# unixpickle/vq-voice-swap

Hardware: AMD Instinct MI355X
Metric: audio clips/sec (whole node), unet64 50-step DDPM on 4s@16kHz waveforms (higher is better)
Workload: dtype fp16; 1 GPU; unet64 50-step DDPM (constrain, schedule t**2), 64 clips/GPU x 1 GPU of T=64000; global_batch=64, parallelism=clips sharded over 1 GPU(s), gather to rank 0

## Files before the change

include/vqvs.h:

```cpp
#ifndef VQVS_H
#define VQVS_H

#include <stdint.h>

#ifdef __cplusplus
extern "C" {
#endif

#define VQVS_OK 0
#define VQVS_ERR_ARG (-1)
#define VQVS_ERR_HIP (-2)
#define VQVS_ERR_STATE (-3)

#define VQVS_KIND_PREDICTOR 0
#define VQVS_KIND_ENCODER 1
#define VQVS_KIND_RESBLOCK 2
#define VQVS_KIND_CLASSIFIER 3
#define VQVS_KIND_ENCPRED 4

#define VQVS_KIND_MFCC_ENCODER 5

#define VQVS_KIND_PREDICTOR_GRAD 6

#define VQVS_PREC_F32 0
#define VQVS_PREC_BF16 1
#define VQVS_PREC_F16 2

typedef struct vqvs_model vqvs_model;

typedef struct vqvs_cfg {
  int32_t kind;
  int32_t base_channels;
  int32_t in_channels;
  int32_t out_channels;
  int32_t cond_channels;
  int32_t num_labels;
  int32_t precision;
  int32_t max_batch;
  int32_t max_T;
  int32_t debug_taps;
  int32_t rb_cin, rb_cout, rb_resize , rb_dilation, rb_emb_channels ;
  int32_t reserved[5];
  int32_t topology_set;
  int32_t n_levels;
  int32_t channel_mult[12];
  int32_t depth_mult;
  int32_t n_dilations;
  int32_t dilations[12];
} vqvs_cfg;
#define VQVS_MAX_LEVELS 12

int vqvs_param_count(const vqvs_cfg* cfg);
int vqvs_param_info(const vqvs_cfg* cfg, int index, char* name_out, int name_cap, int64_t shape_out[4], int* ndim_out);

int vqvs_model_create(const vqvs_cfg* cfg, const float* const* h_params, int n_params, int device, vqvs_model** out);
void vqvs_model_destroy(vqvs_model* m);
int64_t vqvs_model_device_bytes(const vqvs_model* m);

int vqvs_unet_forward(vqvs_model* m, const float* d_x, const float* d_ts, const float* d_cond,
                      const int64_t* d_labels, float* d_out, int B, int T, void* stream);

int vqvs_encoder_forward(vqvs_model* m, const float* d_x, float* d_z, int B, int T, void* stream);

int vqvs_mfcc_encoder_forward(vqvs_model* m, const float* d_x, float* d_z, int B, int T, void* stream);

int vqvs_mfcc_encoder_forward_logmel(vqvs_model* m, const float* d_logmel, float* d_z, int B, int T, void* stream);

int vqvs_resblock_forward(vqvs_model* m, const float* d_x, const float* d_emb, float* d_y, int B, int L, void* stream);

int vqvs_model_status(vqvs_model* m, unsigned* h_status);

int vqvs_classifier_forward(vqvs_model* m, const float* d_x, const float* d_ts, float* d_logits, int B, int T, void* stream);
int vqvs_classifier_guidance(vqvs_model* m, const float* d_x, const float* d_ts, const int64_t* d_labels, float scale,
                             float* d_grad, float* d_logits, int B, int T, void* stream);
int vqvs_classifier_features(vqvs_model* m, const float* d_x, const float* d_ts, float* d_feat,
                             float* d_logits, float* d_probs, int B, int T, void* stream);

int vqvs_feature_moments(const float* d_feat, int B, int F, const float* d_shift, double* d_s1, double* d_s2, void* stream);

int vqvs_encpred_forward(vqvs_model* m, const float* d_x, const float* d_ts, float* d_logits, int B, int T, void* stream);
int vqvs_encpred_guidance(vqvs_model* m, const float* d_x, const float* d_ts, const int64_t* d_targets, float scale,
                          float* d_grad, float* d_logits, int B, int T, void* stream);

int vqvs_unet_embed_grad(vqvs_model* m, const float* d_x_t, const float* d_ts, const float* d_cond, const float* d_vec,
                         const float* d_eps, float* d_mse, float* d_grad, float* d_pred, int B, int T, void* stream);
int vqvs_embed_adamw(float* d_rows, float* d_m, float* d_v, const float* d_grad, const int64_t* d_row_of_clip, int n, int B, int E,
                     int step, float lr, float beta1, float beta2, float eps, float weight_decay, void* stream);

int vqvs_head_xent_grad(const float* d_feat, const float* d_w_old, const float* d_b_old, const float* d_new, const int64_t* d_targets,
                        float* d_act, float* d_logits, double* d_nll, int64_t* d_top1, double* d_new_mass, double* d_coef, int B, int F,
                        int K, int n, void* stream);
int vqvs_head_adamw(float* d_new, float* d_m, float* d_v, const float* d_act, const double* d_coef, int n, int B, int F, int step,
                    float lr, float beta1, float beta2, float eps, float weight_decay, void* stream);

#define VQVS_DDPM_SIGMA_LARGE 1u
#define VQVS_DDPM_CONSTRAIN 2u
int vqvs_ddpm_step(const float* d_x_t, const float* d_eps, const float* d_noise, const float* d_alpha_t,
                   const float* d_alpha_prev, float* d_x_prev, int B, int T, uint32_t flags, float noise_scale,
                   uint64_t seed, uint64_t clip_offset, uint32_t step_index, void* stream);
int vqvs_ddpm_step_windows(const float* d_x, const float* d_eps, const float* d_noise, const float* d_alpha_t,
                           const float* d_alpha_prev, float* d_x_prev, float* d_windows, int n, int W, int H, uint32_t flags,
                           float noise_scale, uint64_t seed, uint64_t clip, uint32_t step_index, void* stream);
int vqvs_ddpm_mean(const float* d_x_t, const float* d_eps, const float* d_alpha_t, const float* d_alpha_prev,
                   float* d_mean, int B, int T, void* stream);
int vqvs_ddpm_guided_eps(const float* d_x_t, const float* d_mean, const float* d_grad, const float* d_alpha_t,
                         const float* d_alpha_prev, float* d_eps_out, int B, int T, uint32_t flags, void* stream);
#define VQVS_DDIM_CONSTRAIN 2u
#define VQVS_DDIM_INVERT 4u
int vqvs_ddim_step(const float* d_x_t, const float* d_eps, const float* d_grad, const float* d_noise, const float* d_alpha_t,
                   const float* d_alpha_to, float* d_x_to, int B, int T, uint32_t flags, float eta, float noise_scale,
                   uint64_t seed, uint64_t clip_offset, uint32_t step_index, void* stream);
int vqvs_ddim_step_windows(const float* d_x, const float* d_eps, const float* d_grad, const float* d_noise, const float* d_alpha_t,
                           const float* d_alpha_to, float* d_x_to, float* d_windows, int n, int W, int H, uint32_t flags, float eta,
                           float noise_scale, uint64_t seed, uint64_t clip, uint32_t step_index, void* stream);
int vqvs_dpmpp_step(const float* d_x_t, const float* d_eps, const float* d_grad, const float* d_x0_prev, const float* d_alpha_from,
                    const float* d_alpha_t, const float* d_alpha_to, float* d_x_to, float* d_x0_out, int B, int T, uint32_t flags,
                    void* stream);
int vqvs_dpmpp_step_windows(const float* d_x, const float* d_eps, const float* d_grad, const float* d_x0_prev, const float* d_alpha_from,
                            const float* d_alpha_t, const float* d_alpha_to, float* d_x_to, float* d_x0_out, float* d_windows, int n, int W,
                            int H, uint32_t flags, void* stream);
int vqvs_keep_region(float* d_x, const float* d_x0, const uint8_t* d_keep, const float* d_noise, const float* d_alpha, int B, int T,
                     float noise_scale, uint64_t seed, uint64_t clip_offset, uint32_t index, void* stream);
int vqvs_keep_region_windows(float* d_x, float* d_windows, const float* d_x0, const uint8_t* d_keep, const float* d_noise,
                             const float* d_alpha, int n, int W, int H, float noise_scale, uint64_t seed, uint64_t clip, uint32_t index,
                             void* stream);
int vqvs_randn(float* d_out, int B, int T, uint64_t seed, uint64_t clip_offset, uint32_t stream_id, void* stream);

int vqvs_ddpm_noise(const float* d_x0, int x0_rows, const float* d_alpha, const float* d_eps, int eps_rows,
                    const int64_t* d_noise_index, float* d_x_t, int B, int T, uint64_t seed, uint64_t clip_offset, void* stream);
int vqvs_ddpm_sqerr(const float* d_pred, const float* d_eps, int eps_rows, const int64_t* d_noise_index, float* d_loss,
                    int B, int T, uint64_t seed, uint64_t clip_offset, void* stream);

int vqvs_vq_argmin(const float* d_z, const float* d_dict, int64_t* d_idx, int B, int Cd, int T1, int K, void* stream);
int vqvs_vq_quantize(const float* d_z, const float* d_dict, int64_t* d_idx, float* d_embedded, double* d_sqerr, int64_t* d_hist,
                     int B, int Cd, int T1, int K, void* stream);
int vqvs_vq_embed(const int64_t* d_idx, const float* d_dict, float* d_out, int B, int Cd, int T1, int K, void* stream);

int vqvs_xent_score(const float* d_logits, const int64_t* d_targets, double* d_nll, int64_t* d_top1, int64_t* d_topk, int k,
                    int64_t* d_confusion, int B, int K, int L, void* stream);

int vqvs_spectral_distance(const float* d_a, const float* d_b, const float* d_window, const double* d_twiddle,
                           const float* d_fb, const float* d_dct, double* d_mcd, double* d_lsd,
                           int B, int T, int n_fft, int hop, int n_mels, int n_ceps, float eps, void* stream);
// ... 27 lines not shown
```

vq_voice_swap_amd/_native.py:

```python

from __future__ import annotations

import ctypes as C
import os
import subprocess
from typing import Dict, List, Optional, Sequence, Tuple

_HERE = os.path.dirname(os.path.abspath(__file__))
LIB_PATH = os.environ.get("VQVS_LIB_PATH") or os.path.join(_HERE, "libvqvs_hip.so")
CSRC = os.path.join(_HERE, "csrc")

KIND_PREDICTOR, KIND_ENCODER, KIND_RESBLOCK, KIND_CLASSIFIER, KIND_ENCPRED, KIND_MFCC_ENCODER, KIND_PREDICTOR_GRAD = 0, 1, 2, 3, 4, 5, 6
PREC_F32, PREC_BF16, PREC_F16 = 0, 1, 2
DDPM_SIGMA_LARGE, DDPM_CONSTRAIN = 1, 2
DDIM_CONSTRAIN, DDIM_INVERT = 2, 4
STREAM_STEP, STREAM_XT, STREAM_LOSS, STREAM_KEEP = 0, 1, 2, 3
PRECISIONS = {"fp32": PREC_F32, "f32": PREC_F32, "float32": PREC_F32, "bf16": PREC_BF16, "bfloat16": PREC_BF16,
              "fp16": PREC_F16, "f16": PREC_F16, "float16": PREC_F16, "half": PREC_F16}


class Cfg(C.Structure):
    _fields_ = [
        ("kind", C.c_int32),
        ("base_channels", C.c_int32),
        ("in_channels", C.c_int32),
        ("out_channels", C.c_int32),
        ("cond_channels", C.c_int32),
        ("num_labels", C.c_int32),
        ("precision", C.c_int32),
        ("max_batch", C.c_int32),
        ("max_T", C.c_int32),
        ("debug_taps", C.c_int32),
        ("rb_cin", C.c_int32),
        ("rb_cout", C.c_int32),
        ("rb_resize", C.c_int32),
        ("rb_dilation", C.c_int32),
        ("rb_emb_channels", C.c_int32),
        ("reserved", C.c_int32 * 5),
        ("topology_set", C.c_int32),
        ("n_levels", C.c_int32),
        ("channel_mult", C.c_int32 * 12),
        ("depth_mult", C.c_int32),
        ("n_dilations", C.c_int32),
        ("dilations", C.c_int32 * 12),
    ]

    def set_topology(self, channel_mult, depth_mult, dilations):
        if len(channel_mult) > 12 or len(dilations) > 12:
            raise ValueError("the gfx950 library builds at most 12 levels and 12 middle / output dilations")
        self.topology_set = 1
        self.n_levels = len(channel_mult)
        for i, m in enumerate(channel_mult):
            self.channel_mult[i] = int(m)
        self.depth_mult = int(depth_mult)
        self.n_dilations = len(dilations)
        for i, d in enumerate(dilations):
            self.dilations[i] = int(d)


EXPORTS = [
    "vqvs_param_count", "vqvs_param_info", "vqvs_model_create", "vqvs_model_destroy", "vqvs_model_device_bytes",
    "vqvs_unet_forward", "vqvs_encoder_forward", "vqvs_mfcc_encoder_forward", "vqvs_mfcc_encoder_forward_logmel", "vqvs_model_status", "vqvs_resblock_forward", "vqvs_classifier_forward",
    "vqvs_classifier_guidance", "vqvs_classifier_features", "vqvs_feature_moments", "vqvs_encpred_forward", "vqvs_encpred_guidance", "vqvs_ddpm_step", "vqvs_ddpm_step_windows", "vqvs_ddim_step", "vqvs_ddim_step_windows", "vqvs_dpmpp_step", "vqvs_dpmpp_step_windows", "vqvs_keep_region", "vqvs_keep_region_windows", "vqvs_ddpm_mean",
    "vqvs_ddpm_guided_eps", "vqvs_randn", "vqvs_ddpm_noise", "vqvs_ddpm_sqerr", "vqvs_vq_argmin", "vqvs_vq_quantize", "vqvs_vq_embed", "vqvs_xent_score", "vqvs_spectral_distance", "vqvs_pitch_distance", "vqvs_debug_tap_count",
    "vqvs_debug_tap_info", "vqvs_debug_tap_rows", "vqvs_debug_read_tap", "vqvs_debug_read_embedding", "vqvs_forward_kernel_count", "vqvs_forward_model_bytes",
    "vqvs_forward_flops", "vqvs_set_profiling", "vqvs_op_info", "vqvs_op_desc", "vqvs_profile_read", "vqvs_last_error", "vqvs_version",
    "vqvs_unet_embed_grad", "vqvs_embed_adamw", "vqvs_debug_read_dfilm", "vqvs_head_xent_grad", "vqvs_head_adamw",
]

_lib = None


class NativeError(RuntimeError):
    pass


class NativeArgumentError(NativeError, ValueError):
    """VQVS_ERR_ARG: the library refused the arguments on the host, before it touched the device.  A ValueError, as the
    reference raises for shape problems, and a NativeError like every other error the library reports."""


def build(force: bool = False, verbose: bool = False) -> str:
    cmd = ["make", "-C", CSRC, "-j", str(min(8, os.cpu_count() or 1))]
    if force:
        subprocess.run(["make", "-C", CSRC, "clean"], check=True, capture_output=not verbose)
    r = subprocess.run(cmd, capture_output=True, text=True)
    if r.returncode != 0:
        raise NativeError("building libvqvs_hip.so failed:\n" + r.stdout[-4000:] + r.stderr[-4000:])
    if verbose:
        print(r.stdout)
    return LIB_PATH


def lib():
    global _lib
    if _lib is not None:
        return _lib
    if not os.path.exists(LIB_PATH):
        raise NativeError(
            f"{LIB_PATH} is missing. Build it with `python -c 'import __graft_entry__ as g; g.build()'` "
            "(or `make -C vq_voice_swap_amd/csrc`). There is no CPU fallback for the sampling hot path."
        )
    if os.environ.get("HIP_FORCE_DEV_KERNARG") is None:
        import warnings

        warnings.warn("HIP_FORCE_DEV_KERNARG is not set: the HIP runtime keeps kernel arguments in host memory and every launch of the "
                      "sampler starts with loads across PCIe (~2 % slower, DESIGN.md section 7).  Set HIP_FORCE_DEV_KERNARG=1 in the "
                      "process environment before the first HIP call (bench.py and the sample_*.py scripts do).", RuntimeWarning, stacklevel=2)
    L = C.CDLL(LIB_PATH)
    vp, i32, i64, u32, u64, f32 = C.c_void_p, C.c_int, C.c_int64, C.c_uint32, C.c_uint64, C.c_float
    L.vqvs_last_error.restype = C.c_char_p
    L.vqvs_version.restype = C.c_char_p
    L.vqvs_param_count.argtypes = [C.POINTER(Cfg)]
    L.vqvs_param_info.argtypes = [C.POINTER(Cfg), i32, C.c_char_p, i32, C.POINTER(i64), C.POINTER(i32)]
    L.vqvs_model_create.argtypes = [C.POINTER(Cfg), C.POINTER(vp), i32, i32, C.POINTER(vp)]
    L.vqvs_model_destroy.argtypes = [vp]
    L.vqvs_model_destroy.restype = None
    L.vqvs_model_device_bytes.argtypes = [vp]
    L.vqvs_model_device_bytes.restype = i64
    L.vqvs_unet_forward.argtypes = [vp, vp, vp, vp, vp, vp, i32, i32, vp]
    L.vqvs_unet_embed_grad.argtypes = [vp, vp, vp, vp, vp, vp, vp, vp, vp, i32, i32, vp]
    L.vqvs_embed_adamw.argtypes = [vp, vp, vp, vp, vp, i32, i32, i32, i32, f32, f32, f32, f32, f32, vp]
    L.vqvs_debug_read_dfilm.argtypes = [vp, i32, vp]
    L.vqvs_head_xent_grad.argtypes = [vp, vp, vp, vp, vp, vp, vp, vp, vp, vp, vp, i32, i32, i32, i32, vp]
    L.vqvs_head_adamw.argtypes = [vp, vp, vp, vp, vp, i32, i32, i32, i32, f32, f32, f32, f32, f32, vp]
    L.vqvs_encoder_forward.argtypes = [vp, vp, vp, i32, i32, vp]
    L.vqvs_mfcc_encoder_forward.argtypes = [vp, vp, vp, i32, i32, vp]
    L.vqvs_mfcc_encoder_forward_logmel.argtypes = [vp, vp, vp, i32, i32, vp]
    L.vqvs_model_status.argtypes = [vp, vp]
    L.vqvs_resblock_forward.argtypes = [vp, vp, vp, vp, i32, i32, vp]
    L.vqvs_classifier_forward.argtypes = [vp, vp, vp, vp, i32, i32, vp]
    L.vqvs_classifier_guidance.argtypes = [vp, vp, vp, vp, f32, vp, vp, i32, i32, vp]
    L.vqvs_classifier_features.argtypes = [vp, vp, vp, vp, vp, vp, i32, i32, vp]
    L.vqvs_feature_moments.argtypes = [vp, i32, i32, vp, vp, vp, vp]
    L.vqvs_encpred_forward.argtypes = [vp, vp, vp, vp, i32, i32, vp]
    L.vqvs_encpred_guidance.argtypes = [vp, vp, vp, vp, f32, vp, vp, i32, i32, vp]
    L.vqvs_ddpm_step.argtypes = [vp, vp, vp, vp, vp, vp, i32, i32, u32, f32, u64, u64, u32, vp]
    L.vqvs_ddpm_step_windows.argtypes = [vp, vp, vp, vp, vp, vp, vp, i32, i32, i32, u32, f32, u64, u64, u32, vp]
    L.vqvs_ddim_step.argtypes = [vp, vp, vp, vp, vp, vp, vp, i32, i32, u32, f32, f32, u64, u64, u32, vp]
    L.vqvs_ddim_step_windows.argtypes = [vp, vp, vp, vp, vp, vp, vp, vp, i32, i32, i32, u32, f32, f32, u64, u64, u32, vp]
    L.vqvs_dpmpp_step.argtypes = [vp, vp, vp, vp, vp, vp, vp, vp, vp, i32, i32, u32, vp]
    L.vqvs_dpmpp_step_windows.argtypes = [vp, vp, vp, vp, vp, vp, vp, vp, vp, vp, i32, i32, i32, u32, vp]
    L.vqvs_keep_region.argtypes = [vp, vp, vp, vp, vp, i32, i32, f32, u64, u64, u32, vp]
    L.vqvs_keep_region_windows.argtypes = [vp, vp, vp, vp, vp, vp, i32, i32, i32, f32, u64, u64, u32, vp]
    L.vqvs_ddpm_mean.argtypes = [vp, vp, vp, vp, vp, i32, i32, vp]
    L.vqvs_ddpm_guided_eps.argtypes = [vp, vp, vp, vp, vp, vp, i32, i32, u32, vp]
    L.vqvs_randn.argtypes = [vp, i32, i32, u64, u64, u32, vp]
    L.vqvs_ddpm_noise.argtypes = [vp, i32, vp, vp, i32, vp, vp, i32, i32, u64, u64, vp]
    L.vqvs_ddpm_sqerr.argtypes = [vp, vp, i32, vp, vp, i32, i32, u64, u64, vp]
    L.vqvs_vq_argmin.argtypes = [vp, vp, vp, i32, i32, i32, i32, vp]
    L.vqvs_vq_quantize.argtypes = [vp, vp, vp, vp, vp, vp, i32, i32, i32, i32, vp]
    L.vqvs_vq_embed.argtypes = [vp, vp, vp, i32, i32, i32, i32, vp]
    L.vqvs_xent_score.argtypes = [vp, vp, vp, vp, vp, i32, vp, i32, i32, i32, vp]
    L.vqvs_spectral_distance.argtypes = [vp, vp, vp, vp, vp, vp, vp, vp, i32, i32, i32, i32, i32, i32, f32, vp]
    L.vqvs_pitch_distance.argtypes = [vp, vp, vp, vp, vp, vp, i32, i32, i32, i32, i32, i32, C.c_double, vp]
    L.vqvs_debug_tap_count.argtypes = [vp]
    L.vqvs_debug_tap_info.argtypes = [vp, i32, C.c_char_p, i32, C.POINTER(i32), C.POINTER(i32)]
    L.vqvs_debug_tap_rows.argtypes = [vp, i32, i32]
    L.vqvs_debug_read_tap.argtypes = [vp, i32, i32, i32, vp]
    L.vqvs_debug_read_embedding.argtypes = [vp, i32, vp]
    L.vqvs_forward_kernel_count.argtypes = [vp]
    L.vqvs_forward_model_bytes.argtypes = [vp, i32, i32]
    L.vqvs_forward_model_bytes.restype = i64
    L.vqvs_forward_flops.argtypes = [vp, i32, i32]
    L.vqvs_forward_flops.restype = i64
    L.vqvs_set_profiling.argtypes = [vp, i32]
    L.vqvs_op_info.argtypes = [vp, i32, C.c_char_p, i32, C.POINTER(i64), C.POINTER(i64), i32, i32]
    L.vqvs_profile_read.argtypes = [vp, vp, i32]
    L.vqvs_op_desc.argtypes = [vp, i32, C.c_char_p, i32]
    _lib = L
    return L


def last_error() -> str:
    return (lib().vqvs_last_error() or b"").decode("utf-8", "replace")


def check(rc: int) -> None:
    if rc == 0:
        return
    msg = last_error()
    if rc == -1:
        if msg.startswith("must provide"):
            raise AssertionError(msg)
        raise NativeArgumentError(msg)
    raise NativeError(f"libvqvs_hip error {rc}: {msg}")


def param_table(cfg: Cfg) -> List[Tuple[str, Tuple[int, ...]]]:
    L = lib()
    n = L.vqvs_param_count(C.byref(cfg))
    if n < 0:
        check(n)
    out = []
    name = C.create_string_buffer(256)
    shape = (C.c_int64 * 4)()
    nd = C.c_int()
    for i in range(n):
        check(L.vqvs_param_info(C.byref(cfg), i, name, 256, shape, C.byref(nd)))
        out.append((name.value.decode(), tuple(int(shape[k]) for k in range(nd.value))))
    return out


# ... 162 lines not shown
```

vq_voice_swap_amd/csrc/api.cpp:

```cpp
#include <cmath>
#include <cstring>
#include <initializer_list>
#include <map>
#include <mutex>
#include <string>
#include <utility>
#include <vector>

#include "net.hpp"
#include "sampler_kernels.hpp"

namespace vqvs {
static thread_local std::string g_err;
void set_error(const std::string& msg) { g_err = msg; }

struct DeviceScratch {
  void* p = nullptr;
  size_t bytes = 0;
  unsigned long long used = 0;
  int leases = 0;
  std::vector<void*> retired;
};
static std::map<std::pair<int, void*>, DeviceScratch> g_scratch;
static std::mutex g_scratch_mu;
// ... 41 lines not shown
      VQVS_HIP(hipFree(sc.p));
      sc.p = nullptr;
      sc.bytes = 0;
    }
  } else if (sc.p && sc.bytes < bytes) {
    sc.retired.push_back(sc.p);
    sc.p = nullptr;
    sc.bytes = 0;
  }
  if (!sc.p) {
    size_t n = bytes < MIN_BYTES ? MIN_BYTES : bytes;
    VQVS_HIP(hipMalloc(&sc.p, n));
    sc.bytes = n;
  }
  sc.used = ++g_scratch_tick;
  ++sc.leases;
  lease.sc = &sc;
  lease.p = sc.p;
  return 0;
}
}

using namespace vqvs;

extern "C" {

const char* vqvs_last_error(void) { return g_err.c_str(); }
#ifndef VQVS_BUILD_ID
#define VQVS_BUILD_ID "unstamped"
#endif
const char* vqvs_version(void) { return "vqvs-hip 0.1 (gfx950) build " VQVS_BUILD_ID; }

int vqvs_param_count(const vqvs_cfg* cfg) {
  if (!cfg) VQVS_FAIL(VQVS_ERR_ARG, "cfg is NULL");
  std::vector<ParamDef> p;
  if (int e = enumerate_params(*cfg, p)) return e;
  return (int)p.size();
}

int vqvs_param_info(const vqvs_cfg* cfg, int index, char* name_out, int name_cap, int64_t shape_out[4], int* ndim_out) {
  if (!cfg) VQVS_FAIL(VQVS_ERR_ARG, "cfg is NULL");
  std::vector<ParamDef> p;
  if (int e = enumerate_params(*cfg, p)) return e;
  if (index < 0 || index >= (int)p.size()) VQVS_FAIL(VQVS_ERR_ARG, "param index %d out of range", index);
  const ParamDef& d = p[index];
  if (name_out && name_cap > 0) {
    strncpy(name_out, d.name.c_str(), name_cap - 1);
    name_out[name_cap - 1] = 0;
  }
  if (shape_out)
    for (int i = 0; i < 4; ++i) shape_out[i] = i < (int)d.shape.size() ? d.shape[i] : 1;
  if (ndim_out) *ndim_out = (int)d.shape.size();
  return 0;
}

int vqvs_model_create(const vqvs_cfg* cfg, const float* const* h_params, int n_params, int device, vqvs_model** out) {
  if (!cfg || !h_params || !out) VQVS_FAIL(VQVS_ERR_ARG, "NULL argument");
  *out = nullptr;
  std::vector<ParamDef> p;
  if (int e = enumerate_params(*cfg, p)) return e;
  if (n_params != (int)p.size()) VQVS_FAIL(VQVS_ERR_ARG, "expected %d parameters, got %d", (int)p.size(), n_params);
  for (int i = 0; i < n_params; ++i)
    if (!h_params[i]) VQVS_FAIL(VQVS_ERR_ARG, "parameter %d (%s) is NULL", i, p[i].name.c_str());
  int ndev = 0;
  VQVS_HIP(hipGetDeviceCount(&ndev));
  if (device < 0 || device >= ndev) VQVS_FAIL(VQVS_ERR_ARG, "device %d not present (%d visible)", device, ndev);
  VQVS_HIP(hipSetDevice(device));
  vqvs_model* m = new vqvs_model();
  m->cfg = *cfg;
  m->device = device;
  if (int e = build_model(m, h_params)) {
    vqvs_model_destroy(m);
    return e;
  }
  *out = m;
  return 0;
}

void vqvs_model_destroy(vqvs_model* m) {
  if (!m) return;
  for (auto e : m->events) (void)hipEventDestroy(e);
  if (m->d_weights) (void)hipFree(m->d_weights);
  if (m->d_arena) (void)hipFree(m->d_arena);
  delete m;
}

int64_t vqvs_model_device_bytes(const vqvs_model* m) { return m ? (int64_t)(m->weights_bytes + m->arena_bytes) : 0; }

static int check_run(vqvs_model* m, int kind, int B, int L) {
  if (!m) VQVS_FAIL(VQVS_ERR_ARG, "model is NULL");
  if (m->cfg.kind != kind) VQVS_FAIL(VQVS_ERR_STATE, "handle kind %d used as kind %d", m->cfg.kind, kind);
  if (B < 1 || B > m->cfg.max_batch) VQVS_FAIL(VQVS_ERR_ARG, "batch %d outside 1..%d", B, m->cfg.max_batch);
  if (L < 1 || L > m->cfg.max_T) VQVS_FAIL(VQVS_ERR_ARG, "length %d outside 1..%d", L, m->cfg.max_T);
  if (kind == VQVS_KIND_CLASSIFIER && (L % (2 * unet_rate(m->cfg))))
    VQVS_FAIL(VQVS_ERR_ARG, "T=%d is not a multiple of the classifier downsample rate %d", L, 2 * unet_rate(m->cfg));
  if (kind != VQVS_KIND_RESBLOCK && kind != VQVS_KIND_MFCC_ENCODER && (L % unet_rate(m->cfg)))
    VQVS_FAIL(VQVS_ERR_ARG, "T=%d is not a multiple of the UNet downsample rate %d", L, unet_rate(m->cfg));
  if (kind == VQVS_KIND_RESBLOCK && m->cfg.rb_resize == RESIZE_AVG2 && (L % 2)) VQVS_FAIL(VQVS_ERR_ARG, "avg-pool resblock needs even L");
  return 0;
}

int vqvs_unet_forward(vqvs_model* m, const float* d_x, const float* d_ts, const float* d_cond, const int64_t* d_labels, float* d_out,
                      int B, int T, void* stream) {
  if (int e = check_run(m, VQVS_KIND_PREDICTOR, B, T)) return e;
  if (!d_x || !d_ts || !d_out) VQVS_FAIL(VQVS_ERR_ARG, "x, ts and out must be non-NULL");
  if ((d_labels == nullptr) != (m->cfg.num_labels == 0)) VQVS_FAIL(VQVS_ERR_ARG, "must provide labels if and only if model is class conditional");
  if ((d_cond == nullptr) != (m->cfg.cond_channels == 0)) VQVS_FAIL(VQVS_ERR_ARG, "must provide cond sequence if and only if model is conditional");
  RunCtx c;
  c.B = B;
  c.Lbase = T;
  c.x = d_x;
  c.ts = d_ts;
  c.cond = d_cond;
  c.labels = d_labels;
  c.out = d_out;
  c.st = reinterpret_cast<hipStream_t>(stream);
  return run_model(m, c);
}

int vqvs_unet_embed_grad(vqvs_model* m, const float* d_x_t, const float* d_ts, const float* d_cond, const float* d_vec, const float* d_eps,
                         float* d_mse, float* d_grad, float* d_pred, int B, int T, void* stream) {
  if (int e = check_run(m, VQVS_KIND_PREDICTOR_GRAD, B, T)) return e;
  if (!d_x_t || !d_ts || !d_vec) VQVS_FAIL(VQVS_ERR_ARG, "x_t, ts and vec must be non-NULL");
  if ((d_cond == nullptr) != (m->cfg.cond_channels == 0)) VQVS_FAIL(VQVS_ERR_ARG, "must provide cond sequence if and only if model is conditional");
  if ((d_mse == nullptr) != (d_grad == nullptr)) VQVS_FAIL(VQVS_ERR_ARG, "mse and grad must be given together (both NULL: the forward alone)");
  const bool backward = d_grad != nullptr;
  if (backward && !d_eps) VQVS_FAIL(VQVS_ERR_ARG, "eps must be non-NULL when mse and grad are asked for");
  if (!backward && !d_pred) VQVS_FAIL(VQVS_ERR_ARG, "nothing to compute: mse, grad and pred are all NULL");
  RunCtx c;
  c.B = B;
  c.Lbase = T;
  c.x = d_x_t;
  c.ts = d_ts;
  c.cond = d_cond;
  c.class_vec = d_vec;
  c.eps = d_eps;
  c.mse = d_mse;
  c.egrad = d_grad;
  c.out = d_pred;
  c.backward = backward;
  c.st = reinterpret_cast<hipStream_t>(stream);
  return run_model(m, c);
}

int vqvs_embed_adamw(float* d_rows, float* d_m, float* d_v, const float* d_grad, const int64_t* d_row_of_clip, int n, int B, int E,
                     int step, float lr, float beta1, float beta2, float eps, float weight_decay, void* stream) {
  if (!d_rows || !d_m || !d_v || !d_grad || !d_row_of_clip) VQVS_FAIL(VQVS_ERR_ARG, "rows, m, v, grad and row_of_clip must be non-NULL");
  if (n < 1 || B < 1 || E < 1) VQVS_FAIL(VQVS_ERR_ARG, "bad shape n=%d B=%d E=%d", n, B, E);
  if (step < 1) VQVS_FAIL(VQVS_ERR_ARG, "step=%d: the count of this step starts at 1", step);
  if (!std::isfinite(lr) || lr < 0.f) VQVS_FAIL(VQVS_ERR_ARG, "lr=%g must be finite and not negative", (double)lr);
  if (!std::isfinite(eps) || eps < 0.f) VQVS_FAIL(VQVS_ERR_ARG, "eps=%g must be finite and not negative", (double)eps);
  if (!std::isfinite(weight_decay) || weight_decay < 0.f) VQVS_FAIL(VQVS_ERR_ARG, "weight_decay=%g must be finite and not negative", (double)weight_decay);
  if (!(beta1 >= 0.f && beta1 < 1.f) || !(beta2 >= 0.f && beta2 < 1.f)) VQVS_FAIL(VQVS_ERR_ARG, "betas (%g, %g) must lie in [0, 1)", (double)beta1, (double)beta2);
  return run_embed_adamw(d_rows, d_m, d_v, d_grad, d_row_of_clip, n, B, E, step, lr, beta1, beta2, eps, weight_decay,
                         reinterpret_cast<hipStream_t>(stream));
}

int vqvs_head_xent_grad(const float* d_feat, const float* d_w_old, const float* d_b_old, const float* d_new, const int64_t* d_targets,
                        float* d_act, float* d_logits, double* d_nll, int64_t* d_top1, double* d_new_mass, double* d_coef, int B, int F,
                        int K, int n, void* stream) {
  if (!d_feat || !d_w_old || !d_b_old || !d_new || !d_targets || !d_nll || !d_coef)
    VQVS_FAIL(VQVS_ERR_ARG, "feat, w_old, b_old, new, targets, nll and coef must be non-NULL");
  if (B < 1 || B > 65535) VQVS_FAIL(VQVS_ERR_ARG, "batch %d outside 1..65535", B);
  if (F < 1 || F > 4096) VQVS_FAIL(VQVS_ERR_ARG, "feature width %d outside 1..4096", F);
  if (K < 1 || n < 1 || K > 8192 || n > 8192 || K + n > 8192) VQVS_FAIL(VQVS_ERR_ARG, "K=%d old and n=%d new labels: each at least 1, together at most 8192", K, n);
  return run_head_xent_grad(d_feat, d_w_old, d_b_old, d_new, d_targets, d_act, d_logits, d_nll, d_top1, d_new_mass, d_coef, B, F, K, n,
                            reinterpret_cast<hipStream_t>(stream));
}

int vqvs_head_adamw(float* d_new, float* d_m, float* d_v, const float* d_act, const double* d_coef, int n, int B, int F, int step,
                    float lr, float beta1, float beta2, float eps, float weight_decay, void* stream) {
  if (!d_new || !d_m || !d_v || !d_act || !d_coef) VQVS_FAIL(VQVS_ERR_ARG, "new, m, v, act and coef must be non-NULL");
  if (n < 1 || B < 1 || F < 1) VQVS_FAIL(VQVS_ERR_ARG, "bad shape n=%d B=%d F=%d", n, B, F);
  if (n > 8192 || B > 65535 || F > 4096) VQVS_FAIL(VQVS_ERR_ARG, "n=%d B=%d F=%d outside 1..8192, 1..65535, 1..4096", n, B, F);
  if (step < 1) VQVS_FAIL(VQVS_ERR_ARG, "step=%d: the count of this step starts at 1", step);
  if (!std::isfinite(lr) || lr < 0.f) VQVS_FAIL(VQVS_ERR_ARG, "lr=%g must be finite and not negative", (double)lr);
  if (!std::isfinite(eps) || eps < 0.f) VQVS_FAIL(VQVS_ERR_ARG, "eps=%g must be finite and not negative", (double)eps);
  if (!std::isfinite(weight_decay) || weight_decay < 0.f) VQVS_FAIL(VQVS_ERR_ARG, "weight_decay=%g must be finite and not negative", (double)weight_decay);
  if (!(beta1 >= 0.f && beta1 < 1.f) || !(beta2 >= 0.f && beta2 < 1.f)) VQVS_FAIL(VQVS_ERR_ARG, "betas (%g, %g) must lie in [0, 1)", (double)beta1, (double)beta2);
  return run_head_adamw(d_new, d_m, d_v, d_act, d_coef, n, B, F, step, lr, beta1, beta2, eps, weight_decay,
                        reinterpret_cast<hipStream_t>(stream));
}

int vqvs_encoder_forward(vqvs_model* m, const float* d_x, float* d_z, int B, int T, void* stream) {
  if (int e = check_run(m, VQVS_KIND_ENCODER, B, T)) return e;
  if (!d_x || !d_z) VQVS_FAIL(VQVS_ERR_ARG, "x and z must be non-NULL");
  RunCtx c;
  c.B = B;
  c.Lbase = T;
  c.x = d_x;
  c.out = d_z;
  c.st = reinterpret_cast<hipStream_t>(stream);
  return run_model(m, c);
}

int vqvs_mfcc_encoder_forward(vqvs_model* m, const float* d_x, float* d_z, int B, int T, void* stream) {
  if (int e = check_run(m, VQVS_KIND_MFCC_ENCODER, B, T)) return e;
  if (!d_x || !d_z) VQVS_FAIL(VQVS_ERR_ARG, "x and z must be non-NULL");
  if (T < 800) VQVS_FAIL(VQVS_ERR_ARG, "T=%d is too short for the MFCC front end (needs at least 800 samples)", T);
// ... 415 lines not shown
  if (!a) VQVS_FAIL(VQVS_ERR_ARG, "a must be non-NULL");
  if (!b && (period_b || counts || sums)) VQVS_FAIL(VQVS_ERR_ARG, "b is NULL: period_b, counts and sums must be NULL too");
  if (!b && !period_a) VQVS_FAIL(VQVS_ERR_ARG, "b is NULL: period_a must be given");
  if (!period_a && !period_b && !counts && !sums) VQVS_FAIL(VQVS_ERR_ARG, "every output is NULL: nothing to compute");
  if (B < 1 || B > 65535) VQVS_FAIL(VQVS_ERR_ARG, "batch %d outside 1..65535", B);
  if (T < 1 || T > (1 << 30)) VQVS_FAIL(VQVS_ERR_ARG, "clip of %d samples outside 1..2^30", T);
  if (window < 16 || window > 2048) VQVS_FAIL(VQVS_ERR_ARG, "window=%d outside 16..2048", window);
  if (hop < 1 || hop > window) VQVS_FAIL(VQVS_ERR_ARG, "hop=%d outside 1..window=%d", hop, window);
  if (T / hop + 1 > (1 << 25)) VQVS_FAIL(VQVS_ERR_ARG, "T=%d at hop=%d is more than 2^25 frames per clip", T, hop);
  if (tau_max < 3 || tau_max > 1023) VQVS_FAIL(VQVS_ERR_ARG, "tau_max=%d outside 3..1023", tau_max);
  if (tau_min < 2 || tau_min >= tau_max) VQVS_FAIL(VQVS_ERR_ARG, "tau_min=%d outside 2..tau_max-1=%d", tau_min, tau_max - 1);
  if ((int64_t)window * tau_max > (1 << 20))
    VQVS_FAIL(VQVS_ERR_ARG, "window=%d times tau_max=%d is more than 2^20: the sums would not stay below 2^53", window, tau_max);
  if (!std::isfinite(threshold) || !(threshold > 0.0) || threshold > 1.0) VQVS_FAIL(VQVS_ERR_ARG, "threshold=%g must lie in (0, 1]", threshold);
  const int64_t N = (int64_t)B * T, NF = (int64_t)B * (T / hop + 1);
  const struct { const void* p; int64_t bytes; const char* name; } outs[] = {
      {period_a, NF * 8, "period_a"}, {period_b, NF * 8, "period_b"}, {counts, (int64_t)B * 32, "counts"}, {sums, (int64_t)B * 16, "sums"}};
  for (const auto& out : outs) {
    if (bytes_overlap(out.p, out.bytes, a, N * 4) || bytes_overlap(out.p, out.bytes, b, N * 4))
      VQVS_FAIL(VQVS_ERR_ARG, "%s must not overlap a or b", out.name);
    for (const auto& other : outs)
      if (&other != &out && bytes_overlap(out.p, out.bytes, other.p, other.bytes))
        VQVS_FAIL(VQVS_ERR_ARG, "%s must not overlap %s", out.name, other.name);
  }
  ScratchLease lease;
  if (counts || sums)
    if (int e = scratch_get(pitch_distance_scratch_bytes(B, T, hop), stream, lease)) return e;
  return run_pitch_distance(a, b, period_a, period_b, counts, sums, lease.p, B, T, window, hop, tau_min, tau_max, threshold,
                            reinterpret_cast<hipStream_t>(stream));
}

int vqvs_vq_embed(const int64_t* d_idx, const float* d_dict, float* d_out, int B, int Cd, int T1, int K, void* stream) {
  if (!d_idx || !d_dict || !d_out) VQVS_FAIL(VQVS_ERR_ARG, "idx, dict and out must be non-NULL");
  if (B < 1 || Cd < 1 || T1 < 1 || K < 1) VQVS_FAIL(VQVS_ERR_ARG, "bad shape B=%d Cd=%d T1=%d K=%d", B, Cd, T1, K);
  if (B > 65535) VQVS_FAIL(VQVS_ERR_ARG, "batch %d outside 1..65535", B);
  if (Cd > 65535) VQVS_FAIL(VQVS_ERR_ARG, "channels %d outside 1..65535", Cd);
  return run_vq_embed(d_idx, d_dict, d_out, B, Cd, T1, K, reinterpret_cast<hipStream_t>(stream));
}

int vqvs_debug_tap_count(const vqvs_model* m) { return m ? (int)m->taps.size() : 0; }

int vqvs_debug_tap_info(const vqvs_model* m, int i, char* name_out, int name_cap, int* channels, int* length_shift) {
  if (!m || i < 0 || i >= (int)m->taps.size()) VQVS_FAIL(VQVS_ERR_ARG, "bad tap index");
  if (name_out && name_cap > 0) {
    strncpy(name_out, m->taps[i].name.c_str(), name_cap - 1);
    name_out[name_cap - 1] = 0;
  }
  if (channels) *channels = m->taps[i].t.C;
  if (length_shift) *length_shift = m->taps[i].t.lshift;
  return 0;
}

int vqvs_debug_tap_rows(const vqvs_model* m, int i, int T) {
  if (!m || i < 0 || i >= (int)m->taps.size()) VQVS_FAIL(VQVS_ERR_ARG, "bad tap index");
  return tensor_rows(T, m->taps[i].t.lshift);
}

int vqvs_debug_read_tap(vqvs_model* m, int i, int B, int T, float* h_out) {
  if (!m || i < 0 || i >= (int)m->taps.size() || !h_out) VQVS_FAIL(VQVS_ERR_ARG, "bad argument");
  if (!m->cfg.debug_taps) VQVS_FAIL(VQVS_ERR_STATE, "model was not created with debug_taps=1");
  const TensorH& t = m->taps[i].t;
  const int L = tensor_rows(T, t.lshift);
  const size_t n = (size_t)B * t.C * L;
  float* d_tmp = nullptr;
  VQVS_HIP(hipSetDevice(m->device));
  VQVS_HIP(hipMalloc(reinterpret_cast<void**>(&d_tmp), n * 4));
  int e = launch_ntc_to_nct(m->d_arena + t.off, d_tmp, B, t.C, L, t.f32 ? 0 : m->cfg.precision, nullptr);
  if (!e) {
    hipError_t he = hipMemcpy(h_out, d_tmp, n * 4, hipMemcpyDeviceToHost);
    if (he != hipSuccess) {
      set_error(std::string("hipMemcpy failed: ") + hipGetErrorString(he));
      e = VQVS_ERR_HIP;
    }
  }
  (void)hipFree(d_tmp);
  return e;
}

int vqvs_debug_read_embedding(vqvs_model* m, int B, float* h_out) {
  if (!m || !h_out || B < 1 || B > m->cfg.max_batch) VQVS_FAIL(VQVS_ERR_ARG, "bad argument");
  if (!m->emb_E) VQVS_FAIL(VQVS_ERR_STATE, "this model kind has no timestep embedding");
  VQVS_HIP(hipSetDevice(m->device));
  VQVS_HIP(hipDeviceSynchronize());
  const float* src = reinterpret_cast<const float*>(m->d_arena + m->misc_off) + m->emb_misc_off;
  VQVS_HIP(hipMemcpy(h_out, src, (size_t)B * m->emb_E * sizeof(float), hipMemcpyDeviceToHost));
  return m->emb_E;
}

int vqvs_debug_read_dfilm(vqvs_model* m, int B, float* h_out) {
  if (!m || !h_out || B < 1 || B > m->cfg.max_batch) VQVS_FAIL(VQVS_ERR_ARG, "bad argument");
  if (!m->dfilm_R) VQVS_FAIL(VQVS_ERR_STATE, "this model kind has no FiLM-gradient buffer");
  VQVS_HIP(hipSetDevice(m->device));
  VQVS_HIP(hipDeviceSynchronize());
  const float* src = reinterpret_cast<const float*>(m->d_arena + m->misc_off) + m->dfilm_misc_off;
  VQVS_HIP(hipMemcpy(h_out, src, (size_t)B * m->dfilm_R * sizeof(float), hipMemcpyDeviceToHost));
  return m->dfilm_R;
}

int vqvs_forward_kernel_count(const vqvs_model* m) { return m ? (int)m->ops.size() : 0; }

int64_t vqvs_forward_model_bytes(const vqvs_model* m, int B, int T) {
  if (!m) return 0;
  const double es = m->cfg.precision == VQVS_PREC_F32 ? 4.0 : 2.0;
  return (int64_t)((m->cost.elems_T * es + m->cost.bytes_f32) * (double)T * (double)B);
}

int64_t vqvs_forward_flops(const vqvs_model* m, int B, int T) {
  if (!m) return 0;
  return (int64_t)(m->cost.flops * (double)T * (double)B);
}

}

extern "C" {

int vqvs_set_profiling(vqvs_model* m, int on) {
  if (!m) VQVS_FAIL(VQVS_ERR_ARG, "model is NULL");
  m->profiling = on != 0;
  return 0;
}

int vqvs_op_info(const vqvs_model* m, int i, char* kind_out, int kind_cap, int64_t* bytes_out, int64_t* flops_out, int B, int T) {
  if (!m || i < 0 || i >= (int)m->meta.size()) VQVS_FAIL(VQVS_ERR_ARG, "bad op index");
  const auto& mt = m->meta[i];
  if (kind_out && kind_cap > 0) {
    strncpy(kind_out, mt.kind.c_str(), kind_cap - 1);
    kind_out[kind_cap - 1] = 0;
  }
  const double es = m->cfg.precision == VQVS_PREC_F32 ? 4.0 : 2.0;
  if (bytes_out) *bytes_out = (int64_t)((mt.elems_T * es + mt.bytes_f32) * (double)T * (double)B);
  if (flops_out) *flops_out = (int64_t)(mt.flops * (double)T * (double)B);
  return 0;
}

int vqvs_op_desc(const vqvs_model* m, int i, char* out, int cap) {
  if (!m || i < 0 || i >= (int)m->meta.size() || !out || cap < 1) VQVS_FAIL(VQVS_ERR_ARG, "bad argument");
  strncpy(out, m->meta[i].desc.c_str(), cap - 1);
  out[cap - 1] = 0;
  return 0;
}

int vqvs_model_status(vqvs_model* m, unsigned* h_status) {
  if (!m || !h_status) VQVS_FAIL(VQVS_ERR_ARG, "NULL argument");
  *h_status = 0;
  if (m->status_misc_off == (size_t)-1) return 0;
  unsigned* d = reinterpret_cast<unsigned*>(reinterpret_cast<float*>(m->d_arena + m->misc_off) + m->status_misc_off);
  VQVS_HIP(hipDeviceSynchronize());
  VQVS_HIP(hipMemcpy(h_status, d, sizeof(unsigned), hipMemcpyDeviceToHost));
  if (*h_status) VQVS_HIP(hipMemset(d, 0, sizeof(unsigned)));
  return 0;
}

int vqvs_profile_read(vqvs_model* m, float* h_ms, int cap) {
  if (!m || !h_ms) VQVS_FAIL(VQVS_ERR_ARG, "NULL argument");
  if (m->events.size() != m->ops.size() + 1) VQVS_FAIL(VQVS_ERR_STATE, "no profiled forward has run");
  VQVS_HIP(hipEventSynchronize(m->events.back()));
  const int n = (int)m->ops.size() < cap ? (int)m->ops.size() : cap;
  for (int i = 0; i < n; ++i) VQVS_HIP(hipEventElapsedTime(&h_ms[i], m->events[i], m->events[i + 1]));
  return n;
}

}

#ifdef VQVS_TIMING
namespace vqvs { int conv_timing_read(unsigned long long* out16, int reset); }
extern "C" int vqvs_debug_conv_timing(unsigned long long* h_out16, int reset) { return vqvs::conv_timing_read(h_out16, reset); }
// ... 4 lines not shown
```

vq_voice_swap_amd/csrc/kernels.hpp:

```cpp
#pragma once

#include "common.hpp"

namespace vqvs {

enum { RESIZE_NONE = 0, RESIZE_AVG2 = 1, RESIZE_UP2 = 2 };

struct SegDesc {
  const void* src;
  const float2* ss;
  long long w_off;
  int Csrc;
  int c0;
  int C;
  int Lsrc;
  int ntaps;
  int dil;
  int resize;
  int ss_stride, ss_c0;
  const void* src2;
  const float4* coef;
  int coef_stride, coef_c0;
};

// ... 9 lines not shown
  const bf16_t* w_hi;
  const bf16_t* w_lo;
  long long w_bytes;
  const float* bias;
  int Cout, Lout;
  const void* skip;
  int skip_C, skip_L, skip_resize;
  void* out;
  int out_f32;
  float* stats;
  int ntiles;
  int tile_rows;
  int out_rows;
  int epi_gelu;
  BwActFuse bw[2];
  int nbw;
  const float2* bw_ss;
  int bw_ss_stride;
  const GnArgs* gn;
  int ws_f32;
  int rev;
};

int launch_conv(const ConvArgs& a, int B, int precision, hipStream_t st);
int launch_conv_ws(const ConvArgs& a, int B, int precision, hipStream_t st);
bool ws_fuses_gn(const ConvArgs& a, int B, int precision);
bool ws_available(int precision);
int conv_tile_rows(int dmax, int Cout, int precision, bool ws_ok = false);

struct InConvArgs {
  const float* x;
  const float* w;
  int Cin;
  const float* bias;
  const void* condp;
  int cond_len;
  void* out;
  float* stats;
  int C, T, ntiles;
};
int launch_in_conv(const InConvArgs& a, int B, int precision, hipStream_t st);

struct OutConvArgs {
  const void* in;
  const float2* ss;
  const float* w;
  float bias;
  float* out;
  int C, L;
};
int launch_out_conv(const OutConvArgs& a, int B, int precision, hipStream_t st);

struct GnSrc {
  const float* partials;
  int ntiles, C;
};
struct GnArgs {
  GnSrc src[2];
  int nsrc, Ctot, groups;
  double inv_count;
  const float* gamma;
  const float* beta;
  const float* film;
  int film_stride, film_off;
  float2* ss;
  float2* mr;
  unsigned* status;
  int guard;
};
int launch_gn_prepare(const GnArgs& a, int B, hipStream_t st);

struct TimeEmbedArgs {
  const float* ts;
  const float* freqs;
  const float *w1, *b1;
  const float *w2, *b2;
  const float* class_embed;
  const int64_t* labels;
  const float* class_vec;
  int num_labels;
  float* emb;
  float* gemb;
  int E;
};
int launch_time_embed(const TimeEmbedArgs& a, int B, hipStream_t st);
int launch_gelu_rows(const float* in, float* out, int n, hipStream_t st);

struct FilmArgs {
  const float* gemb;
  const float* w;
  const float* bias;
  float* film;
  int E, R;
};
int launch_film(const FilmArgs& a, int B, hipStream_t st);

struct XformArgs {
  const void* in;
  const float2* ss;
  void* out;
  int C, Lin, Lout, avg, ss_stride, ss_c0;
};
int launch_xform(const XformArgs& a, int B, int precision, hipStream_t st);

enum { BW_SAME = 0, BW_FROM_HALF = 1, BW_FROM_DOUBLE = 2 };
struct BwActArgs {
  const void* t;
  const void* xf;
  const float2* ss;
  void* du;
  float* partials;
  int C, L, resize;
  int t_C, t_c0, du_C, du_c0, ss_stride, ss_c0, part_C, part_c0;
};
int launch_bw_act(const BwActArgs& a, int B, int precision, hipStream_t st);

struct GnBwArgs {
  const float* partials;
  int ntiles, C, groups;
  double inv_count;
  const float2* ss;
  const float2* mr;
  float4* coef;
};
int launch_gn_bw(const GnBwArgs& a, int B, hipStream_t st);

struct BwAffineArgs {
  const void* du;
  const void* xf;
  const float4* coef;
  const void* skip;
  int skip_mode;
  const void* extra;
  void* out;
  int C, L;
  int du_C, du_c0, coef_stride, coef_c0, extra_C, extra_c0;
};
int launch_bw_affine(const BwAffineArgs& a, int B, int precision, hipStream_t st);
int launch_bw_add(const void* a, const void* b, void* out, long long n, int precision, hipStream_t st);

struct InConvBwArgs {
  const void* dh;
  const float* w;
  float* out;
  int C, T;
  float out_scale;
};
int launch_in_conv_bw(const InConvBwArgs& a, int B, int precision, hipStream_t st);

int mse_head_scratch_doubles(int B, int T);
int run_mse_head(const float* pred, const float* eps, float* dout, float* mse, double* scratch, int B, int T, hipStream_t st);

struct OutConvBwArgs {
  const float* dout;
  const void* xf;
  const float2* ss;
  const float* w;
  void* du;
  float* partials;
  int C, L;
};
int launch_out_conv_bw(const OutConvBwArgs& a, int B, hipStream_t st);

struct FilmGradArgs {
  const void* du;
  const void* h1;
// ... 104 lines not shown
```

vq_voice_swap_amd/csrc/misc_kernels.hip:

```cpp
#include <atomic>

#include "kernels.hpp"

namespace vqvs {

namespace {

template <typename T, bool MC>
__global__ __launch_bounds__(256) void in_conv_kernel(const InConvArgs a) {
  __shared__ float red[256 * 8 * 2];
  const int tid = threadIdx.x;
  const int b = blockIdx.y;
  const int t0 = blockIdx.x * STAT_TILE;
  const int opr = a.C >> 3;
  const int rpp = 256 / opr;
  const int oct = tid % opr;
  const int r0 = tid / opr;
  const int c = oct * 8;
  float w0[8], w1[8], w2[8], bs[8];
  const int Cin = MC ? a.Cin : 1;
#pragma unroll
  for (int j = 0; j < 8; ++j) {
    w0[j] = a.w[(c + j) * Cin * 3 + 0];
    w1[j] = a.w[(c + j) * Cin * 3 + 1];
    w2[j] = a.w[(c + j) * Cin * 3 + 2];
    bs[j] = a.bias[c + j];
  }
  const float* xb = a.x + (size_t)b * Cin * a.T;
  f32x8 s1 = f32x8_zero(), s2 = f32x8_zero();
  const bool active = r0 < rpp && oct < opr;
  const float cond_scale = a.condp ? (float)a.cond_len / (float)a.T : 0.f;
  if (active) {
    for (int r = r0; r < STAT_TILE; r += rpp) {
      const int t = t0 + r;
      if (t >= a.T) break;
      const float xm = t > 0 ? xb[t - 1] : 0.f;
      const float x0 = xb[t];
      const float xp = t + 1 < a.T ? xb[t + 1] : 0.f;
      f32x8 v;
#pragma unroll
      for (int j = 0; j < 8; ++j) v[j] = fmaf(w2[j], xp, fmaf(w1[j], x0, fmaf(w0[j], xm, bs[j])));
      if constexpr (MC)
      for (int ci = 1; ci < Cin; ++ci) {
        const float* xc = xb + (size_t)ci * a.T;
        const float ym = t > 0 ? xc[t - 1] : 0.f, y0 = xc[t], yp = t + 1 < a.T ? xc[t + 1] : 0.f;
#pragma unroll
        for (int j = 0; j < 8; ++j) {
          const float* wc = a.w + ((c + j) * Cin + ci) * 3;
          v[j] = fmaf(wc[2], yp, fmaf(wc[1], y0, fmaf(wc[0], ym, v[j])));
        }
      }
      if (a.condp) {
        const int cr = min((int)floorf((float)t * cond_scale), a.cond_len - 1);
        const T* cp = reinterpret_cast<const T*>(a.condp) + ((size_t)b * a.cond_len + cr) * a.C + c;
        v += Elem<T>::load8(cp);
      }
      s1 += v;
      s2 += v * v;
      Elem<T>::store8(reinterpret_cast<T*>(a.out) + ((size_t)b * a.T + t) * a.C + c, v);
    }
  }
  if (active) {
#pragma unroll
    for (int j = 0; j < 8; ++j) {
      red[(r0 * a.C + c + j) * 2 + 0] = s1[j];
      red[(r0 * a.C + c + j) * 2 + 1] = s2[j];
    }
  }
  __syncthreads();
  if (tid < a.C) {
    float t1 = 0.f, t2 = 0.f;
    for (int g = 0; g < rpp; ++g) {
      t1 += red[(g * a.C + tid) * 2 + 0];
      t2 += red[(g * a.C + tid) * 2 + 1];
    }
    float* o = a.stats + (((size_t)b * a.ntiles + blockIdx.x) * a.C + tid) * 2;
    o[0] = t1;
    o[1] = t2;
  }
}

template <typename T>
__global__ __launch_bounds__(256) void out_conv_kernel(const OutConvArgs a) {
  constexpr int GQ = GeluQ<T>::q;
  __shared__ float y[3][STAT_TILE + 2];
  const int tid = threadIdx.x;
  const int b = blockIdx.y;
  const int t0 = blockIdx.x * STAT_TILE;
  const int opr = a.C >> 3;
  const int rpp = 256 / opr;
  const int oct = tid % opr;
  const int r0 = tid / opr;
  const int c = oct * 8;
  f32x8 sc, sh, w0, w1, w2;
  {
    const float2* p = a.ss + (size_t)b * a.C + c;
#pragma unroll
    for (int j = 0; j < 8; ++j) {
      const float2 q = p[j];
      sc[j] = q.x;
      sh[j] = q.y;
      w0[j] = a.w[0 * a.C + c + j];
      w1[j] = a.w[1 * a.C + c + j];
      w2[j] = a.w[2 * a.C + c + j];
    }
  }
  const T* xb = reinterpret_cast<const T*>(a.in) + (size_t)b * a.L * a.C + c;
  for (int r = r0; r < STAT_TILE + 2; r += rpp) {
    const int t = t0 - 1 + r;
    float p0 = 0.f, p1 = 0.f, p2 = 0.f;
    if (t >= 0 && t < a.L) {
      const f32x8 v = Elem<T>::load8(xb + (size_t)t * a.C);
#pragma unroll
      for (int j = 0; j < 8; j += 2) {
        const f32x2 g = gelu2<GQ>(fma2(f32x2{v[j], v[j + 1]}, f32x2{sc[j], sc[j + 1]}, f32x2{sh[j], sh[j + 1]}));
        p0 = fmaf(w0[j + 1], g[1], fmaf(w0[j], g[0], p0));
        p1 = fmaf(w1[j + 1], g[1], fmaf(w1[j], g[0], p1));
        p2 = fmaf(w2[j + 1], g[1], fmaf(w2[j], g[0], p2));
      }
    }
    for (int m = 1; m < opr; m <<= 1) {
      p0 += __shfl_xor(p0, m);
      p1 += __shfl_xor(p1, m);
      p2 += __shfl_xor(p2, m);
    }
    if (oct == 0) {
      y[0][r] = p0;
      y[1][r] = p1;
      y[2][r] = p2;
    }
  }
  __syncthreads();
  const int t = t0 + tid;
  if (t < a.L) a.out[(size_t)b * a.L + t] = a.bias + y[0][tid] + y[1][tid + 1] + y[2][tid + 2];
}

template <typename T>
__global__ __launch_bounds__(256) void out_conv_rows_kernel(const OutConvArgs a) {
  constexpr int GQ = GeluQ<T>::q;
  __shared__ float y[3][STAT_TILE + 2];
  const int tid = threadIdx.x;
  const int b = blockIdx.y;
  const int t0 = blockIdx.x * STAT_TILE;
  const float2* ss = a.ss + (size_t)b * a.C;
  for (int r = tid; r < STAT_TILE + 2; r += 256) {
    const int t = t0 - 1 + r;
    float p0 = 0.f, p1 = 0.f, p2 = 0.f;
    if (t >= 0 && t < a.L) {
      const T* xr = reinterpret_cast<const T*>(a.in) + ((size_t)b * a.L + t) * a.C;
      for (int c = 0; c < a.C; c += 8) {
        const f32x8 v = Elem<T>::load8(xr + c);
#pragma unroll
        for (int j = 0; j < 8; j += 2) {
          const float2 q0 = ss[c + j], q1 = ss[c + j + 1];
          const f32x2 g = gelu2<GQ>(fma2(f32x2{v[j], v[j + 1]}, f32x2{q0.x, q1.x}, f32x2{q0.y, q1.y}));
          p0 = fmaf(a.w[0 * a.C + c + j + 1], g[1], fmaf(a.w[0 * a.C + c + j], g[0], p0));
          p1 = fmaf(a.w[1 * a.C + c + j + 1], g[1], fmaf(a.w[1 * a.C + c + j], g[0], p1));
          p2 = fmaf(a.w[2 * a.C + c + j + 1], g[1], fmaf(a.w[2 * a.C + c + j], g[0], p2));
        }
      }
    }
// ... 37 lines not shown
    unsigned bad = 0;
    if (sl < nsl) {
      const bool second = c >= C0;
      const GnSrc g = second ? a.src[1] : a.src[0];
      const int cl = second ? c - C0 : c;
      const float* p = g.partials + (size_t)b * g.ntiles * g.C * 2;
      for (int t0 = sl; t0 < g.ntiles; t0 += 8 * nsl) {
        float2 q[8];
#pragma unroll
        for (int k = 0; k < 8; ++k) {
          const int t = t0 + k * nsl;
          q[k] = t < g.ntiles ? *reinterpret_cast<const float2*>(p + ((size_t)t * g.C + cl) * 2) : float2{0.f, 0.f};
        }
#pragma unroll
        for (int k = 0; k < 8; ++k) {
          s1 += (double)q[k].x;
          s2 += (double)q[k].y;
          if (!(fabsf(q[k].x) <= 3.0e38f) || !(q[k].y <= 3.0e38f)) bad |= 1u;
          if (a.guard && q[k].y >= 9.0e8f) bad |= 2u;
        }
      }
      part[tid * 2] = s1;
      part[tid * 2 + 1] = s2;
    }
    if (bad && a.status) atomicOr(a.status, bad);
    __syncthreads();
    int top = 1;
    while (top < nsl) top <<= 1;
    for (int st = top >> 1; st >= 1; st >>= 1) {
      if (sl < st && sl + st < nsl) {
        part[tid * 2] += part[(tid + st * cw) * 2];
        part[tid * 2 + 1] += part[(tid + st * cw) * 2 + 1];
      }
      __syncthreads();
    }
    if (tid < cw) {
      chs[c0 + tid] = part[tid * 2];
      chq[c0 + tid] = part[tid * 2 + 1];
    }
    __syncthreads();
  }
  if (tid < ng) {
    double t1 = 0.0, t2 = 0.0;
    for (int j = 0; j < gs; ++j) {
      t1 += chs[tid * gs + j];
      t2 += chq[tid * gs + j];
    }
    const double mean = t1 * a.inv_count;
    double var = t2 * a.inv_count - mean * mean;
    if (var < 0.0) var = 0.0;
    gmean[tid] = mean;
    grstd[tid] = 1.0 / sqrt(var + 1e-5);
  }
  __syncthreads();
  for (int i = tid; i < cw_tot; i += 256) {
    const int c = c_lo + i;
    const int g = i / gs;
    const bool pre = i == tid;
    double scale = grstd[g] * (double)(pre ? pg : a.gamma[c]);
    double shift = (double)(pre ? pb : a.beta[c]) - gmean[g] * scale;
    if (a.film) {
      const float* f = a.film + (size_t)b * a.film_stride + a.film_off;
      const double fa = (double)(pre ? pfa : f[c]) + 1.0;
      const double fb = (double)(pre ? pfb : f[a.Ctot + c]);
      scale *= fa;
      shift = shift * fa + fb;
    }
    a.ss[(size_t)b * a.Ctot + c] = make_float2((float)scale, (float)shift);
    if (a.mr) a.mr[(size_t)b * a.Ctot + c] = make_float2((float)gmean[g], (float)grstd[g]);
  }
}

__device__ __forceinline__ float wave_sum(float v) {
#pragma unroll
  for (int m = 32; m >= 1; m >>= 1) v += __shfl_xor(v, m);
  return v;
}

__global__ __launch_bounds__(256) void time_embed_kernel(const TimeEmbedArgs a) {
  __shared__ float e0[1024], e1[1024];
  const int tid = threadIdx.x;
  const int b = blockIdx.x;
  const int E = a.E, half = E >> 1;
  const float t = a.ts[b];
  for (int j = tid; j < half; j += 256) {
    const float arg = t * a.freqs[j];
    e0[j] = cosf(arg);
    e0[half + j] = sinf(arg);
  }
  __syncthreads();
  for (int r = tid; r < E; r += 256) {
    float acc0 = 0.f, acc1 = 0.f, acc2 = 0.f, acc3 = 0.f;
    for (int j = 0; j < E; j += 4) {
      acc0 = fmaf(a.w1[(size_t)(j + 0) * E + r], e0[j + 0], acc0);
      acc1 = fmaf(a.w1[(size_t)(j + 1) * E + r], e0[j + 1], acc1);
      acc2 = fmaf(a.w1[(size_t)(j + 2) * E + r], e0[j + 2], acc2);
      acc3 = fmaf(a.w1[(size_t)(j + 3) * E + r], e0[j + 3], acc3);
    }
    e1[r] = gelu_f((acc0 + acc1) + (acc2 + acc3) + a.b1[r]);
  }
  __syncthreads();
  const float* ce = nullptr;
  if (a.class_embed) {
    long long lab = a.labels[b];
    if (lab < 0) lab = 0;
    if (lab >= a.num_labels) lab = a.num_labels - 1;
    ce = a.class_embed + (size_t)lab * E;
  }
  for (int r = tid; r < E; r += 256) {
    float acc0 = 0.f, acc1 = 0.f, acc2 = 0.f, acc3 = 0.f;
    for (int j = 0; j < E; j += 4) {
      acc0 = fmaf(a.w2[(size_t)(j + 0) * E + r], e1[j + 0], acc0);
      acc1 = fmaf(a.w2[(size_t)(j + 1) * E + r], e1[j + 1], acc1);
      acc2 = fmaf(a.w2[(size_t)(j + 2) * E + r], e1[j + 2], acc2);
      acc3 = fmaf(a.w2[(size_t)(j + 3) * E + r], e1[j + 3], acc3);
    }
    float v = (acc0 + acc1) + (acc2 + acc3) + a.b2[r];
    if (ce) v += ce[r];
    if (a.class_vec) v += a.class_vec[(size_t)b * E + r];
    a.emb[(size_t)b * E + r] = v;
    a.gemb[(size_t)b * E + r] = gelu_f(v);
  }
}

__global__ void gelu_rows_kernel(const float* in, float* out, int n) {
  const int i = blockIdx.x * 256 + threadIdx.x;
  if (i < n) out[i] = gelu_f(in[i]);
}

constexpr int FILM_NB = 32;
__global__ __launch_bounds__(256) void film_kernel(const FilmArgs a, int B) {
  extern __shared__ __attribute__((aligned(16))) float fsm[];
  float* const g = fsm;
  float* const red = fsm + a.E * FILM_NB;
  const int lane = threadIdx.x & 63, wv = threadIdx.x >> 6;
  const int r = blockIdx.x * 64 + lane;
  const int E = a.E, b0 = blockIdx.y * FILM_NB;
  const int nb = min(FILM_NB, B - b0);
  for (int i = threadIdx.x; i < E * FILM_NB; i += 256) {
    const int e = i / FILM_NB, bb = i % FILM_NB;
    g[i] = bb < nb ? a.gemb[(size_t)(b0 + bb) * E + e] : 0.f;
  }
  __syncthreads();
  float acc[FILM_NB];
#pragma unroll
  for (int k = 0; k < FILM_NB; ++k) acc[k] = 0.f;
  const int eq = E / 4;
  if (r < a.R) {
    for (int e0 = wv * eq; e0 < (wv + 1) * eq; e0 += 8) {
      float w[8];
#pragma unroll
      for (int u = 0; u < 8; ++u) w[u] = a.w[(size_t)(e0 + u) * a.R + r];
#pragma unroll
      for (int u = 0; u < 8; ++u) {
        const f32x4* gp = reinterpret_cast<const f32x4*>(&g[(e0 + u) * FILM_NB]);
#pragma unroll
        for (int q = 0; q < FILM_NB / 4; ++q) {
          const f32x4 gv = gp[q];
          acc[4 * q + 0] = fmaf(w[u], gv[0], acc[4 * q + 0]);
          acc[4 * q + 1] = fmaf(w[u], gv[1], acc[4 * q + 1]);
          acc[4 * q + 2] = fmaf(w[u], gv[2], acc[4 * q + 2]);
          acc[4 * q + 3] = fmaf(w[u], gv[3], acc[4 * q + 3]);
        }
      }
    }
  }
  if (wv > 0) {
#pragma unroll
    for (int k = 0; k < FILM_NB; ++k) red[((wv - 1) * 64 + lane) * (FILM_NB + 1) + k] = acc[k];
  }
  __syncthreads();
  if (wv == 0 && r < a.R) {
    const float bias = a.bias[r];
#pragma unroll
    for (int k = 0; k < FILM_NB; ++k) {
      float v = acc[k];
#pragma unroll
      for (int w2 = 0; w2 < 3; ++w2) v += red[(w2 * 64 + lane) * (FILM_NB + 1) + k];
      if (k < nb) a.film[(size_t)(b0 + k) * a.R + r] = v + bias;
    }
  }
}

template <typename T>
__global__ __launch_bounds__(256) void xform_kernel(const XformArgs a) {
  constexpr int GQ = GeluQ<T>::q;
  const int b = blockIdx.y;
  const int opr = a.C >> 3;
  const long long item = (long long)blockIdx.x * 256 + threadIdx.x;
  if (item >= (long long)a.Lout * opr) return;
  const int t = (int)(item / opr), c = (int)(item % opr) * 8;
  f32x8 sc, sh;
  const float2* p = a.ss + (size_t)b * a.ss_stride + a.ss_c0 + c;
#pragma unroll
  for (int j = 0; j < 8; ++j) {
    const float2 q = p[j];
    sc[j] = q.x;
    sh[j] = q.y;
  }
  const T* in = reinterpret_cast<const T*>(a.in) + (size_t)b * a.Lin * a.C + c;
  auto tr = [&](f32x8 v) {
    f32x8 r;
#pragma unroll
    for (int j = 0; j < 8; j += 2) {
      const f32x2 g = gelu2<GQ>(fma2(f32x2{v[j], v[j + 1]}, f32x2{sc[j], sc[j + 1]}, f32x2{sh[j], sh[j + 1]}));
      r[j] = g[0];
      r[j + 1] = g[1];
    }
    return r;
  };
  f32x8 v;
  if (a.avg) {
    v = (tr(Elem<T>::load8(in + (size_t)(2 * t) * a.C)) + tr(Elem<T>::load8(in + (size_t)(2 * t + 1) * a.C))) * 0.5f;
  } else {
    v = tr(Elem<T>::load8(in + (size_t)t * a.C));
  }
  Elem<T>::store8(reinterpret_cast<T*>(a.out) + ((size_t)b * a.Lout + t) * a.C + c, v);
}

template <typename T>
__global__ __launch_bounds__(256) void nct_to_ntc_kernel(const float* in, T* out, int C, int L) {
  __shared__ float tile[32][33];
  const int b = blockIdx.z, c0 = blockIdx.y * 32, t0 = blockIdx.x * 32;
  const int tx = threadIdx.x & 31, ty = threadIdx.x >> 5;
  for (int i = ty; i < 32; i += 8) {
    const int c = c0 + i, t = t0 + tx;
    tile[i][tx] = (c < C && t < L) ? in[((size_t)b * C + c) * L + t] : 0.f;
  }
  __syncthreads();
  for (int i = ty; i < 32; i += 8) {
    const int t = t0 + i, c = c0 + tx;
    if (t < L && c < C) out[((size_t)b * L + t) * C + c] = (T)tile[tx][i];
  }
}

template <typename T>
__global__ __launch_bounds__(256) void ntc_to_nct_kernel(const T* in, float* out, int C, int L) {
  __shared__ float tile[32][33];
  const int b = blockIdx.z, c0 = blockIdx.y * 32, t0 = blockIdx.x * 32;
  const int tx = threadIdx.x & 31, ty = threadIdx.x >> 5;
  for (int i = ty; i < 32; i += 8) {
    const int t = t0 + i, c = c0 + tx;
    tile[i][tx] = (c < C && t < L) ? (float)in[((size_t)b * L + t) * C + c] : 0.f;
  }
  __syncthreads();
  for (int i = ty; i < 32; i += 8) {
    const int c = c0 + i, t = t0 + tx;
    if (t < L && c < C) out[((size_t)b * C + c) * L + t] = tile[tx][i];
  }
}

template <typename T>
__global__ __launch_bounds__(256) void ntc_stats_kernel(const T* in, float* stats, int C, int L, int ntiles) {
  const int b = blockIdx.y, tile = blockIdx.x;
  const T* p = in + (size_t)b * L * C;
  for (int c = threadIdx.x; c < C; c += 256) {
    float s1 = 0.f, s2 = 0.f;
    const int t1 = min(L, (tile + 1) * STAT_TILE);
    for (int t = tile * STAT_TILE; t < t1; ++t) {
      const float v = (float)p[(size_t)t * C + c];
      s1 += v;
      s2 += v * v;
    }
    float* o = stats + (((size_t)b * ntiles + tile) * C + c) * 2;
    o[0] = s1;
    o[1] = s2;
  }
}

}

int launch_in_conv(const InConvArgs& a, int B, int precision, hipStream_t st) {
  if (a.C % 8 || a.C > 256) VQVS_FAIL(-1, "in_conv: unsupported C=%d", a.C);
  dim3 grid((a.T + STAT_TILE - 1) / STAT_TILE, B);
  if (a.Cin > 1) {
    VQVS_BY_PRECISION(precision, hipLaunchKernelGGL((in_conv_kernel<T, true>), grid, dim3(256), 0, st, a));
  } else {
    VQVS_BY_PRECISION(precision, hipLaunchKernelGGL((in_conv_kernel<T, false>), grid, dim3(256), 0, st, a));
  }
  VQVS_HIP(hipGetLastError());
  return 0;
}

int launch_out_conv(const OutConvArgs& a, int B, int precision, hipStream_t st) {
  const int opr = a.C / 8;
  if (a.C % 8 || opr > 64) VQVS_FAIL(-1, "out_conv: unsupported C=%d", a.C);
  dim3 grid((a.L + STAT_TILE - 1) / STAT_TILE, B);
  if (opr & (opr - 1)) {
    VQVS_BY_PRECISION(precision, hipLaunchKernelGGL(out_conv_rows_kernel<T>, grid, dim3(256), 0, st, a));
  } else {
    VQVS_BY_PRECISION(precision, hipLaunchKernelGGL(out_conv_kernel<T>, grid, dim3(256), 0, st, a));
  }
  VQVS_HIP(hipGetLastError());
  return 0;
}

int launch_gn_prepare(const GnArgs& a, int B, hipStream_t st) {
  if (a.Ctot > 2048 || a.groups > 32 || a.Ctot % a.groups) VQVS_FAIL(-1, "gn: unsupported Ctot=%d groups=%d", a.Ctot, a.groups);
  int split = GN_SPLIT;
  while (split > 1 && (a.groups % split || (a.groups / split) * (a.Ctot / a.groups) > 256)) split >>= 1;
  if ((a.groups / split) * (a.Ctot / a.groups) > 256 && a.Ctot > 256) split = a.groups;
  hipLaunchKernelGGL(gn_prepare_kernel, dim3(B, split), dim3(256), 0, st, a);
  VQVS_HIP(hipGetLastError());
  return 0;
}

int launch_time_embed(const TimeEmbedArgs& a, int B, hipStream_t st) {
  if (a.E > 1024 || a.E % 64) VQVS_FAIL(-1, "time_embed: unsupported E=%d", a.E);
  hipLaunchKernelGGL(time_embed_kernel, dim3(B), dim3(256), 0, st, a);
  VQVS_HIP(hipGetLastError());
  return 0;
}

int launch_gelu_rows(const float* in, float* out, int n, hipStream_t st) {
  hipLaunchKernelGGL(gelu_rows_kernel, dim3((n + 255) / 256), dim3(256), 0, st, in, out, n);
  VQVS_HIP(hipGetLastError());
  return 0;
}

int launch_film(const FilmArgs& a, int B, hipStream_t st) {
  if (a.E > 1024 || a.E < 32 || a.E % 32) VQVS_FAIL(-1, "film: unsupported E=%d", a.E);
  const int lds = (a.E * FILM_NB + 3 * 64 * (FILM_NB + 1)) * 4;
  static std::atomic<bool> attr_done[64];
  int dev = 0;
  if (hipGetDevice(&dev) != hipSuccess || dev < 0 || dev >= 64) dev = 0;
  if (!attr_done[dev].load(std::memory_order_acquire)) {
    VQVS_HIP(hipFuncSetAttribute(reinterpret_cast<const void*>(&film_kernel), hipFuncAttributeMaxDynamicSharedMemorySize, 160 * 1024));
    attr_done[dev].store(true, std::memory_order_release);
  }
  hipLaunchKernelGGL(film_kernel, dim3((a.R + 63) / 64, (B + FILM_NB - 1) / FILM_NB), dim3(256), lds, st, a, B);
  VQVS_HIP(hipGetLastError());
  return 0;
}

int launch_xform(const XformArgs& a, int B, int precision, hipStream_t st) {
  if (a.C % 8) VQVS_FAIL(-1, "xform: unsupported C=%d", a.C);
  const long long items = (long long)a.Lout * (a.C / 8);
  dim3 grid((unsigned)((items + 255) / 256), B);
  VQVS_BY_PRECISION(precision, hipLaunchKernelGGL(xform_kernel<T>, grid, dim3(256), 0, st, a));
  VQVS_HIP(hipGetLastError());
  return 0;
}

int launch_nct_to_ntc(const float* in, void* out, float* stats, int B, int C, int L, int ntiles, int precision, hipStream_t st) {
  dim3 grid((L + 31) / 32, (C + 31) / 32, B);
  VQVS_BY_PRECISION(precision, {
    hipLaunchKernelGGL(nct_to_ntc_kernel<T>, grid, dim3(256), 0, st, in, (T*)out, C, L);
    if (stats) hipLaunchKernelGGL(ntc_stats_kernel<T>, dim3(ntiles, B), dim3(256), 0, st, (const T*)out, stats, C, L, ntiles);
  });
  VQVS_HIP(hipGetLastError());
  return 0;
}

int launch_ntc_to_nct(const void* in, float* out, int B, int C, int L, int in_precision, hipStream_t st) {
  dim3 grid((L + 31) / 32, (C + 31) / 32, B);
  VQVS_BY_PRECISION(in_precision, hipLaunchKernelGGL(ntc_to_nct_kernel<T>, grid, dim3(256), 0, st, (const T*)in, out, C, L));
  VQVS_HIP(hipGetLastError());
  return 0;
}

}
```

vq_voice_swap_amd/csrc/net.cpp:

```cpp
#include "net.hpp"

#include <algorithm>
#include <cmath>
#include <cstring>
#include <functional>
#include <memory>

namespace vqvs {

namespace {

struct Topo {
  std::vector<int> mult;
  int depth = 2;
  std::vector<int> dil;
  int levels() const { return (int)mult.size(); }
};
Topo topo_of(const vqvs_cfg& c) {
  Topo t;
  const bool custom = c.topology_set != 0 && (c.kind == VQVS_KIND_PREDICTOR || c.kind == VQVS_KIND_PREDICTOR_GRAD || c.kind == VQVS_KIND_ENCODER ||
                                              c.kind == VQVS_KIND_CLASSIFIER);
  if (custom) {
    t.mult.assign(c.channel_mult, c.channel_mult + std::max(0, std::min(c.n_levels, (int)VQVS_MAX_LEVELS)));
    t.depth = c.depth_mult;
// ... 229 lines not shown
    sizes_[t.id] = bytes;
    offs_[t.id] = t.off;
    refs_[t.id] = 1;
    if (stats) {
      t.has_stats = true;
      t.stats_off = stats_floats;
      stats_floats += (size_t)maxB_ * ntiles_of(shiftL(maxL_, lshift), MIN_TILE_ROWS) * C * 2;
      tile_rows_[t.id] = STAT_TILE;
    }
    return t;
  }
  int stat_rows(const TensorH& t) const { return tile_rows_.at(t.id); }
  void retain(const TensorH& t) { refs_[t.id]++; }
  void release(const TensorH& t) {
    if (persist) return;
    if (--refs_[t.id] == 0 && !m_->cfg.debug_taps) arena_free(offs_[t.id], sizes_[t.id]);
  }
  bool persist = false;
  size_t alloc_stats(int C, int lshift) {
    const size_t off = stats_floats;
    stats_floats += (size_t)maxB_ * ntiles_of(shiftL(maxL_, lshift), MIN_TILE_ROWS) * C * 2;
    return off;
  }
  struct BlockRec {
    BlockSpec s;
    TensorH x, x2, h1, out;
    size_t ss1 = 0, ss2 = 0, mr1 = 0, mr2 = 0;
  };
  size_t alloc_ss(int C) {
    const size_t off = ss_floats;
    ss_floats += (size_t)maxB_ * C * 2;
    return off;
  }
  size_t alloc_misc(size_t floats) {
    const size_t off = misc_floats;
    misc_floats += (floats + 63) & ~(size_t)63;
    return off;
  }
  size_t status_off() {
    if (status_off_ == (size_t)-1) {
      status_off_ = alloc_misc(64);
      m_->status_misc_off = status_off_;
    }
    return status_off_;
  }
  size_t status_off_ = (size_t)-1;

  char* act(size_t off) const { return m_->d_arena + off; }
  float* statp(size_t foff) const { return reinterpret_cast<float*>(m_->d_arena + m_->stats_off) + foff; }
  float* ssp(size_t foff) const { return reinterpret_cast<float*>(m_->d_arena + m_->ss_off) + foff; }
  float* miscp(size_t foff) const { return reinterpret_cast<float*>(m_->d_arena + m_->misc_off) + foff; }
  char* wp(size_t off) const { return m_->d_weights + off; }

  struct GnLink {
    std::function<bool(const RunCtx&)> fused;
    std::function<void(const RunCtx&, GnArgs&)> fill;
  };
  std::shared_ptr<GnLink> add_gn(const std::vector<TensorH>& srcs, const std::string& gn_name, bool film, int film_off, int film_stride,
              size_t film_misc_off, size_t ss_off, bool want_mr = false, size_t mr_off = 0) {
    int Ctot = 0;
    for (auto& s : srcs) Ctot += s.C;
    const size_t g_off = blob_f32(gn_name + ".weight");
    const size_t b_off = blob_f32(gn_name + ".bias");
    const int Creal = (int)((long long)Ctot * real_base(m_->cfg) / m_->cfg.base_channels);
    const int groups = gn_groups(Creal);
    const int lshift = srcs[0].lshift;
    Builder* self = this;
    std::vector<TensorH> S = srcs;
    std::vector<int> SR;
    for (auto& t : srcs) SR.push_back(stat_rows(t));
    const size_t st_off = status_off();
    const int guard = m_->cfg.precision == VQVS_PREC_F16 ? 1 : 0;
    m_->meta.push_back({"gn_prepare", gn_name + " C=" + std::to_string(Ctot) + " L>>" + std::to_string(lshift), 0, 0, 0});
    auto link = std::make_shared<GnLink>();
    link->fill = [=](const RunCtx& c, GnArgs& a) {
      const int L = shiftL(c.Lbase, lshift);
      a.nsrc = (int)S.size();
      for (int i = 0; i < a.nsrc; ++i) a.src[i] = GnSrc{self->statp(S[i].stats_off), ntiles_of(L, SR[i]), S[i].C};
      a.Ctot = Ctot;
      a.groups = groups;
      a.inv_count = 1.0 / ((double)(Creal / groups) * (double)L);
      a.gamma = reinterpret_cast<const float*>(self->wp(g_off));
      a.beta = reinterpret_cast<const float*>(self->wp(b_off));
      a.film = film ? self->miscp(film_misc_off) : nullptr;
      a.film_stride = film_stride;
      a.film_off = film_off;
      a.ss = reinterpret_cast<float2*>(self->ssp(ss_off));
      a.mr = want_mr ? reinterpret_cast<float2*>(self->ssp(mr_off)) : nullptr;
      a.status = reinterpret_cast<unsigned*>(self->miscp(st_off));
      a.guard = guard;
    };
    m_->add_op([=](const RunCtx& c) -> int {
      if (link->fused && link->fused(c)) return 0;
      GnArgs a{};
      link->fill(c, a);
      return launch_gn_prepare(a, c.B, c.st);
    });
    return link;
  }

  TensorH add_xform(const TensorH& src, size_t ss_off, int ss_stride, int ss_c0, bool avg) {
    TensorH g = new_tensor(src.C, src.lshift + (avg ? 1 : 0), false, false);
    Builder* self = this;
    const int prec = m_->cfg.precision;
    const TensorH S = src;
    m_->meta.push_back({"xform", "C=" + std::to_string(src.C) + " L>>" + std::to_string(g.lshift) + (avg ? " avg" : ""),
                        src.C * (lscale(src.lshift) + lscale(g.lshift)), 0, 0});
    m_->add_op([=](const RunCtx& c) -> int {
      XformArgs a{};
      a.in = self->act(S.off);
      a.ss = reinterpret_cast<const float2*>(self->ssp(ss_off));
      a.out = self->act(g.off);
      a.C = S.C;
      a.Lin = shiftL(c.Lbase, S.lshift);
      a.Lout = shiftL(c.Lbase, g.lshift);
      a.avg = avg ? 1 : 0;
      a.ss_stride = ss_stride;
      a.ss_c0 = ss_c0;
      return launch_xform(a, c.B, prec, c.st);
    });
    return g;
  }

  struct SegSpec {
    TensorH t;
    int c0, C, ntaps, dil, resize;
    bool xform;
    size_t ss_off;
    int ss_stride, ss_c0;
    long long w_off;
    bool aff2 = false;
    TensorH t2{};
    size_t coef_off = 0;
  };

  struct BwFuse {
    std::vector<TensorH> xf;
    size_t ss_off;
    int ss_stride;
    size_t part_off;
  };
  static bool bw_fuse_enabled() {
    static int v = -1;
    if (v < 0) {
      const char* e = getenv("VQVS_BW_FUSE");
      v = e ? atoi(e) : 1;
    }
    return v != 0;
  }

  int add_conv(const std::vector<SegSpec>& segs, const PackedConv& pk, const std::vector<float>& bias, int Cout, const TensorH& out,
               const TensorH* skip, int skip_resize, int out_lshift = -1000, bool epi_gelu = false, const BwFuse* fuse = nullptr,
               std::shared_ptr<GnLink> gn = nullptr) {
    const size_t hi_off = blob.add(pk.hi.data(), pk.hi.size() * 2);
    const size_t lo_off = m_->cfg.precision == VQVS_PREC_F32 ? blob.add(pk.lo.data(), pk.lo.size() * 2) : 0;
    const size_t bias_off = blob.add(bias.data(), bias.size() * 4);
    const long long w_bytes = (long long)pk.hi.size() * 2;
    const bool x3 = m_->cfg.precision == VQVS_PREC_F32;
    const int prec = m_->cfg.precision;
    Builder* self = this;
    std::vector<SegSpec> S = segs;
    const TensorH O = out;
    const bool has_skip = skip != nullptr;
    const TensorH K = skip ? *skip : TensorH{};
    int dmax = 0;
    for (auto& g : segs)
      if (g.ntaps == 3 && g.dil > dmax) dmax = g.dil;
    int kchunks = skip ? 2 : 0;
// ... 652 lines not shown
  } else if (c.kind == VQVS_KIND_CLASSIFIER) {
    if (c.num_labels < 1 || c.num_labels > 8192) VQVS_FAIL(VQVS_ERR_ARG, "classifier num_labels must be in 1..8192 (got %d)", c.num_labels);
    if (c.max_T % (2 * unet_rate(c))) VQVS_FAIL(VQVS_ERR_ARG, "classifier max_T must be a multiple of %d (got %d)", 2 * unet_rate(c), c.max_T);
    if (c.reserved[1] < 0 || c.reserved[1] * c.base_channels > 4096) VQVS_FAIL(VQVS_ERR_ARG, "classifier output_mult (reserved[1]) out of range (got %d)", c.reserved[1]);
    if (c.topology_set && c.n_dilations != 0) VQVS_FAIL(VQVS_ERR_ARG, "the classifier stem has no dilation list");
  } else {
    if (c.out_channels % 32 || c.out_channels < 32) VQVS_FAIL(VQVS_ERR_ARG, "encoder out_channels must be a multiple of 32");
  }
  return 0;
}

int build_model(vqvs_model* m, const float* const* hp) {
  const vqvs_cfg& c = m->cfg;
  if (int e = check_cfg(c)) return e;
  if (int e = enumerate_params(c, m->params)) return e;
  const int prec = c.precision;
  const int base = c.base_channels;
  const int in_ch = c.in_channels;
  auto keep = std::make_shared<Builder>(m, hp);
  m->keepalive = keep;
  Builder* bp = keep.get();
  Builder& b = *bp;

  if (c.kind == VQVS_KIND_RESBLOCK) {
    BlockSpec s{"", c.rb_cin, c.rb_cout, c.rb_resize, c.rb_dilation, false};
    const int E = c.rb_emb_channels;
    TensorH x = b.new_tensor(c.rb_cin, 0, false, true);
    const int Cin = c.rb_cin;
    m->meta.push_back({"nct_to_ntc", "", 0, 0, 0});
    m->add_op([=](const RunCtx& r) -> int {
      return launch_nct_to_ntc(r.x, bp->act(x.off), bp->statp(x.stats_off), r.B, Cin, r.Lbase, ntiles_of(r.Lbase), prec, r.st);
    });
    size_t film_misc = 0;
    if (E) {
      const size_t gemb = b.alloc_misc((size_t)c.max_batch * E);
      film_misc = b.alloc_misc((size_t)c.max_batch * 2 * c.rb_cout);
      const size_t w_off = b.blob_f32_transposed(b.P("cond_layers.1.weight"), 2 * c.rb_cout, E);
      const size_t bias_off = b.blob_f32("cond_layers.1.bias");
      const int R = 2 * c.rb_cout;
      m->meta.push_back({"film", "", 0, 0, 0});
      m->add_op([=](const RunCtx& r) -> int {
        if (!r.emb) VQVS_FAIL(VQVS_ERR_ARG, "resblock handle was built with an embedding; d_emb is NULL");
        if (int e = launch_gelu_rows(r.emb, bp->miscp(gemb), r.B * E, r.st)) return e;
        FilmArgs f{bp->miscp(gemb), reinterpret_cast<const float*>(bp->wp(w_off)), reinterpret_cast<const float*>(bp->wp(bias_off)),
                   bp->miscp(film_misc), E, R};
        return launch_film(f, r.B, r.st);
      });
    }
    TensorH y = b.resblock("", s, {x}, E != 0, 0, 2 * c.rb_cout, film_misc);
    const int Cout = c.rb_cout;
    m->meta.push_back({"ntc_to_nct", "", 0, 0, 0});
    m->add_op([=](const RunCtx& r) -> int {
      return launch_ntc_to_nct(bp->act(y.off), r.out, r.B, Cout, shiftL(r.Lbase, y.lshift), prec, r.st);
    });
    b.tap("out", y);
  } else if (c.kind == VQVS_KIND_PREDICTOR || c.kind == VQVS_KIND_ENCPRED || c.kind == VQVS_KIND_PREDICTOR_GRAD) {
    const bool encpred = c.kind == VQVS_KIND_ENCPRED;
    const bool gradk = c.kind == VQVS_KIND_PREDICTOR_GRAD;
    const bool keep_bw = encpred || gradk;
    const std::string px = encpred ? "unet." : "";
    b.persist = keep_bw;
    const int E = 4 * base;
    std::vector<BlockSpec> d, mdl, u;
    predictor_blocks(base, topo_of(c), d, mdl, u);
    for (auto* v : {&d, &mdl, &u})
      for (auto& sp : *v) sp.prefix = px + sp.prefix;
    std::vector<float> freqs(E / 2, 0.0f);
    {
      const int Er = 4 * real_base(c);
      const PadMap pm = pad_map(real_base(c));
      for (int i = 0; i < Er / 2; ++i)
        freqs[pm.phys(i)] = (float)(std::exp((double)(float)(-std::log(100.0 / 0.1)) * (double)i / (double)(Er / 2 - 1))) * 100.0f;
    }
    const size_t freq_off = b.blob.add(freqs.data(), freqs.size() * 4);
    const size_t w1 = b.blob_f32_transposed(b.P(px + "time_embed.proj.weight"), E, E), b1 = b.blob_f32(px + "time_embed.proj.bias");
    const size_t w2 = b.blob_f32_transposed(b.P(px + "time_embed_extra.1.weight"), E, E), b2 = b.blob_f32(px + "time_embed_extra.1.bias");
    const size_t ce = c.num_labels > 0 && !gradk ? b.blob_f32(px + "class_embed.weight") : 0;
    const size_t emb_off = b.alloc_misc((size_t)c.max_batch * E);
    const size_t gemb_off = b.alloc_misc((size_t)c.max_batch * E);
    m->emb_misc_off = emb_off;
    m->emb_E = E;
    const int NL = c.num_labels;
    m->meta.push_back({"time_embed", "", 0, 0, 0});
    m->add_op([=](const RunCtx& r) -> int {
      TimeEmbedArgs a{};
      a.ts = r.ts;
      a.freqs = reinterpret_cast<const float*>(bp->wp(freq_off));
      a.w1 = reinterpret_cast<const float*>(bp->wp(w1));
      a.b1 = reinterpret_cast<const float*>(bp->wp(b1));
      a.w2 = reinterpret_cast<const float*>(bp->wp(w2));
      a.b2 = reinterpret_cast<const float*>(bp->wp(b2));
      a.class_embed = NL > 0 && !gradk ? reinterpret_cast<const float*>(bp->wp(ce)) : nullptr;
      a.labels = r.labels;
      a.class_vec = gradk ? r.class_vec : nullptr;
      a.num_labels = NL;
      a.emb = bp->miscp(emb_off);
      a.gemb = bp->miscp(gemb_off);
      a.E = E;
      return launch_time_embed(a, r.B, r.st);
    });
    std::vector<const BlockSpec*> all;
    for (auto& s : d) all.push_back(&s);
    for (auto& s : mdl) all.push_back(&s);
    for (auto& s : u) all.push_back(&s);
    std::vector<int> film_row(all.size());
    int R = 0;
    std::vector<float> Wall, ball;
    for (size_t i = 0; i < all.size(); ++i) {
      film_row[i] = R;
      const float* W = b.P(all[i]->prefix + ".cond_layers.1.weight");
      const float* bb = b.P(all[i]->prefix + ".cond_layers.1.bias");
      const int rows = 2 * all[i]->cout;
      Wall.insert(Wall.end(), W, W + (size_t)rows * E);
      ball.insert(ball.end(), bb, bb + rows);
      R += rows;
    }
    const size_t wall_off = b.blob_f32_transposed(Wall.data(), R, E);
    const size_t ball_off = b.blob.add(ball.data(), ball.size() * 4);
    const size_t film_off = b.alloc_misc((size_t)c.max_batch * R);
    m->meta.push_back({"film", "", 0, 0, 0});
    m->add_op([=](const RunCtx& r) -> int {
      FilmArgs f{bp->miscp(gemb_off), reinterpret_cast<const float*>(bp->wp(wall_off)), reinterpret_cast<const float*>(bp->wp(ball_off)),
                 bp->miscp(film_off), E, R};
      return launch_film(f, r.B, r.st);
    });
    TensorH condp{};
    const bool has_cond = c.cond_channels > 0;
    if (has_cond) {
      const int cond_ls = c.reserved[3] >= LEN_ABS ? c.reserved[3] : (c.reserved[3] == 1 ? LEN_HALF : 8);
      TensorH ct = b.new_tensor(c.cond_channels, cond_ls, false, false);
      const int CC = c.cond_channels;
      m->meta.push_back({"nct_to_ntc", "", 0, 0, 0});
      m->add_op([=](const RunCtx& r) -> int {
        return launch_nct_to_ntc(r.cond, bp->act(ct.off), nullptr, r.B, CC, shiftL(r.Lbase, cond_ls), 0, prec, r.st);
      });
      condp = b.new_tensor(base, cond_ls, false, false);
      PackedConv pk(prec);
      Builder::SegSpec g{ct, 0, CC, 3, 1, RESIZE_NONE, false, 0, 0, 0, 0};
      g.w_off = pk.append(b.P(px + "cond_proj.weight"), base, CC, 3, 0, CC);
      const float* bb = b.P(px + "cond_proj.bias");
      b.add_conv({g}, pk, std::vector<float>(bb, bb + base), base, condp, nullptr, 0);
      b.release(ct);
    }
    TensorH h = b.new_tensor(base, 0, false, true);
    {
      const size_t w = b.blob_f32(px + "in_conv.weight"), bi = b.blob_f32(px + "in_conv.bias");
      const TensorH cp = condp;
      m->meta.push_back({"in_conv", std::to_string(in_ch) + "->" + std::to_string(base), base + (has_cond ? base * lscale(condp.lshift) : 0.0), 4.0 * in_ch, 0});
      m->add_op([=](const RunCtx& r) -> int {
        InConvArgs a{};
        a.x = r.x;
        a.Cin = in_ch;
        a.w = reinterpret_cast<const float*>(bp->wp(w));
        a.bias = reinterpret_cast<const float*>(bp->wp(bi));
        a.condp = has_cond ? bp->act(cp.off) : nullptr;
        a.cond_len = has_cond ? shiftL(r.Lbase, cp.lshift) : 0;
        a.out = bp->act(h.off);
        a.stats = bp->statp(h.stats_off);
        a.C = base;
        a.T = r.Lbase;
        a.ntiles = ntiles_of(r.Lbase);
        return launch_in_conv(a, r.B, prec, r.st);
      });
    }
    if (has_cond) b.release(condp);
    b.tap("in_conv", h);
    std::vector<TensorH> skips{h};
    b.retain(h);
    size_t bi = 0;
    std::vector<Builder::BlockRec> recs(all.size());
    auto recp = [&](size_t i) { return keep_bw ? &recs[i] : nullptr; };
    for (auto& s : d) {
      TensorH o = b.resblock(s.prefix, s, {h}, true, film_row[bi], R, film_off, recp(bi));
      ++bi;
      b.release(h);
      h = o;
      skips.push_back(h);
      b.retain(h);
      b.tap(s.prefix, h);
    }
    for (auto& s : mdl) {
      TensorH o = b.resblock(s.prefix, s, {h}, true, film_row[bi], R, film_off, recp(bi));
      ++bi;
      b.release(h);
      h = o;
      b.tap(s.prefix, h);
    }
    for (auto& s : u) {
      TensorH o;
      if (s.cat) {
        TensorH sk = skips.back();
        skips.pop_back();
        o = b.resblock(s.prefix, s, {h, sk}, true, film_row[bi], R, film_off, recp(bi));
        b.release(sk);
      } else {
        o = b.resblock(s.prefix, s, {h}, true, film_row[bi], R, film_off, recp(bi));
      }
      ++bi;
      b.release(h);
      h = o;
      b.tap(s.prefix, h);
    }
    const size_t ss = b.alloc_ss(base);
    const size_t mr_out = keep_bw ? b.alloc_ss(base) : 0;
    b.add_gn({h}, px + "out.0.0", false, 0, 0, 0, ss, keep_bw, mr_out);
    if (c.out_channels == 1) {
      const float* W = b.P(px + "out.1.weight");
      std::vector<float> wt(3 * base);
// ... 523 lines not shown
```

vq_voice_swap_amd/csrc/net.hpp:

```cpp
#pragma once

#include <functional>
#include <map>
#include <memory>
#include <string>
#include <vector>

#include "../../include/vqvs.h"
#include "kernels.hpp"

namespace vqvs {

struct ParamDef {
  std::string name;
  std::vector<int64_t> shape;
  size_t numel() const {
    size_t n = 1;
    for (auto s : shape) n *= (size_t)s;
    return n;
  }
};

struct TensorH {
  int id = -1;
  size_t off = 0;
  int C = 0;
  int lshift = 0;
  bool f32 = false;
  size_t stats_off = 0;
  bool has_stats = false;
};

struct RunCtx {
  int B = 0;
  int Lbase = 0;
  const float* x = nullptr;
  const float* ts = nullptr;
  const float* cond = nullptr;
  const int64_t* labels = nullptr;
  const float* emb = nullptr;
  const float* logmel = nullptr;
  float* out = nullptr;
  bool backward = false;
  float gscale = 1.0f;
  float* grad_out = nullptr;
  float* feat = nullptr;
  float* probs = nullptr;
  const float* class_vec = nullptr;
  const float* eps = nullptr;
  float* mse = nullptr;
  float* egrad = nullptr;
  hipStream_t st = nullptr;
};

struct TapDef {
  std::string name;
  TensorH t;
};

}

struct vqvs_model {
  vqvs_cfg cfg{};
  int device = 0;
  std::vector<vqvs::ParamDef> params;
  char* d_weights = nullptr;
  size_t weights_bytes = 0;
  char* d_arena = nullptr;
  size_t arena_bytes = 0;
  size_t act_bytes = 0, stats_off = 0, stats_floats = 0, ss_off = 0, ss_floats = 0, misc_off = 0, misc_floats = 0;
  std::vector<std::function<int(const vqvs::RunCtx&)>> ops;
  struct OpMeta {
    std::string kind;
    std::string desc;
    double elems_T = 0;
    double bytes_f32 = 0;
    double flops = 0;
  };
  std::vector<OpMeta> meta;
  std::vector<uint8_t> op_phase;
  int cur_phase = 0;
  void add_op(std::function<int(const vqvs::RunCtx&)> fn) {
    ops.push_back(std::move(fn));
    op_phase.push_back((uint8_t)cur_phase);
  }
  bool profiling = false;
  std::vector<hipEvent_t> events;
  std::vector<vqvs::TapDef> taps;
  struct Cost {
    double elems_T = 0;
    double bytes_f32 = 0;
    double flops = 0;
  } cost;
  int last_B = 0, last_L = 0;
  size_t status_misc_off = (size_t)-1;
  size_t emb_misc_off = 0;
  int emb_E = 0;
  size_t dfilm_misc_off = 0;
  int dfilm_R = 0;
  std::shared_ptr<void> keepalive;
};

namespace vqvs {
int enumerate_params(const vqvs_cfg& cfg, std::vector<ParamDef>& out);
int build_model(vqvs_model* m, const float* const* h_params);
int run_model(vqvs_model* m, const RunCtx& ctx);
int gn_groups(int ch);
int real_base(const vqvs_cfg& c);
int padded_base(int real);
int unet_rate(const vqvs_cfg& cfg);
int tensor_rows(int Lbase, int lshift);
}
```

vq_voice_swap_amd/diffusion.py:

```python

from __future__ import annotations

import contextlib
import math
import operator
from typing import Callable, List, Optional, Sequence, Union

import torch

from . import _native


class Schedule:
    def __call__(self, t: torch.Tensor) -> torch.Tensor:
        raise NotImplementedError


class ExpSchedule(Schedule):

    def __init__(self, alpha_final: float = 1e-5):
        self.alpha_final = alpha_final
        self.k = -math.log(alpha_final)

    def __call__(self, t: torch.Tensor) -> torch.Tensor:
        return torch.exp(-self.k * (t ** 2))


class CosSchedule(Schedule):

    def __call__(self, t: torch.Tensor) -> torch.Tensor:
        return torch.cos(t * math.pi / 2) ** 2


def make_schedule(name: str) -> Schedule:
    if name == "exp":
        return ExpSchedule()
    if name == "cos":
        return CosSchedule()
    raise ValueError(f"unknown schedule: {name}")


def _rows(v: torch.Tensor, like: torch.Tensor) -> torch.Tensor:
    return v.to(like).reshape(-1, *([1] * (like.dim() - 1)))


NoiseSource = Union[None, Sequence[torch.Tensor], Callable[[int], torch.Tensor]]

FEW_GUIDED_STEPS = 10


def _native_modules(fn) -> list:
    seen, out = set(), []

    def add(m):
        if m is not None and hasattr(m, "precision_override") and id(m) not in seen:
            seen.add(id(m))
            out.append(m)

    add(fn)
    add(getattr(fn, "func", None))
    add(getattr(fn, "__self__", None))
    add(getattr(getattr(fn, "func", None), "__self__", None))
    for m in getattr(fn, "native_modules", ()) or ():
        add(m)
    return out


def predictor_check_status(predictor):
    chk = getattr(predictor, "check_status", None)
    if chk is None:
        mods = _native_modules(predictor)
        chk = mods[0].check_status if mods else None
    return chk


def fresh_seed() -> int:
    return int(torch.randint(0, 2 ** 62, (1,)).item())


def _progress(its: range, progress: bool):
    if not progress:
        return its
    from tqdm.auto import tqdm

    return tqdm(its, total=len(its))


def few_guided_steps_promotion(what: str, steps: int, predictor, cond_fn, stacklevel: int = 3):
    if cond_fn is None or steps >= FEW_GUIDED_STEPS:
        return None
    promote = [m for m in _native_modules(predictor) + _native_modules(cond_fn) if getattr(m, "precision", "fp32") != "fp32"]
    if not promote:
        return None
    import os
    import warnings

    modes = sorted({m.precision for m in promote})
    if os.environ.get("VQVS_FEW_STEP_PROMOTE", "1") == "0":
        warnings.warn(f"{what}: {steps} guided steps in the {modes} mode(s) are outside the 1e-3 waveform contract "
                      f"(fewer than {FEW_GUIDED_STEPS} steps); VQVS_FEW_STEP_PROMOTE=0 keeps the mode", RuntimeWarning, stacklevel=stacklevel)
        return None
    warnings.warn(f"{what}: {steps} guided steps (fewer than {FEW_GUIDED_STEPS}): predictor / guidance model run in the fp32 "
                  f"mode for this call (their {modes} mode(s) do not hold the 1e-3 waveform contract at so few steps)",
                  RuntimeWarning, stacklevel=stacklevel)
    stack = contextlib.ExitStack()
    for m in promote:
        stack.enter_context(m.precision_override("fp32"))
    return stack


SAMPLERS = ("ddpm", "ddim", "dpmpp")


def check_sampler(sampler: str, eta: float = 0.0) -> str:
    if sampler not in SAMPLERS:
        raise ValueError(f"sampler={sampler!r}: expected one of {SAMPLERS}")
    if sampler == "ddpm" and eta:
        raise ValueError(f"eta={eta!r} has no meaning for sampler='ddpm' (the DDIM sampler at eta = 1 is its small-sigma step)")
    if sampler == "dpmpp" and eta:
        raise ValueError(f"eta={eta!r} has no meaning for sampler='dpmpp': the DPM-Solver++(2M) sampler is deterministic")
    return sampler


def pick_sampler(diffusion, sampler: str, eta: float = 0.0, *, sigma_large: Optional[bool] = None, windows: bool = False):
    fn = getattr(diffusion, check_sampler(sampler, eta) + ("_sample_windows" if windows else "_sample"))
    if sampler == "ddim":
        return fn, dict(eta=eta)
    if sampler == "dpmpp":
        return fn, {}
    return fn, {} if sigma_large is None else dict(sigma_large=sigma_large)


def warn_few_unguided_steps(what: str, steps: int, predictor, cond_fn, stacklevel: int = 3) -> None:
    if cond_fn is not None or steps >= FEW_GUIDED_STEPS:
        return
    modes = sorted({m.precision for m in _native_modules(predictor) if getattr(m, "precision", "fp32") != "fp32"})
    if modes:
        import warnings

        warnings.warn(f"{what}: {steps} steps (fewer than {FEW_GUIDED_STEPS}) in the {modes} mode(s): the 1e-3 waveform contract is not "
                      "established for so few steps; the mode is kept", RuntimeWarning, stacklevel=stacklevel)


def strength_to_start_step(strength: float, steps: int) -> int:
    strength, steps = float(strength), int(steps)
    if not 0.0 < strength <= 1.0:
        raise ValueError(f"strength={strength!r} must lie in (0, 1]")
    if steps < 1:
# ... 182 lines not shown
            out = torch.empty_like(x)
            _native.check(L.vqvs_ddpm_step(x.data_ptr(), eps.data_ptr(), _native._ptr(noise), a_t.data_ptr(), a_prev.data_ptr(),
                                           out.data_ptr(), B, T, flags, float(noise_scale), int(seed), int(clip_offset),
                                           int(step_index), st))
        return out.view_as(x_t)

    def step_tables(self, steps: int, B: int, schedule: Optional[Callable], device):
        rows = []
        for t in [(i + 1) / steps for i in range(steps)][::-1]:
            ts = torch.tensor([t] * B, dtype=torch.float32)
            t_step = 1 / steps
            if schedule is not None:
                t_step = schedule(ts) - schedule(ts - 1 / steps)
                ts = schedule(ts)
            step = t_step if torch.is_tensor(t_step) else torch.full_like(ts, float(t_step))
            rows.append((ts, self.schedule(ts), self.schedule(ts - step), ts - step))
        return tuple(torch.stack([r[k] for r in rows]).to(torch.float32).contiguous().to(device) for k in range(4))

    @staticmethod
    def check_sample(predictor, x_t: torch.Tensor, what: str) -> None:
        chk = predictor_check_status(predictor)
        if chk is not None:
            chk()
            if not bool(torch.isfinite(x_t).all()):
                raise _native.NativeError(f"{what}: the sample holds non-finite values (a non-finite x_T, conditioning tensor or "
                                          "guidance gradient, or an overflow the range guard reported as a warning)")

    def keep_region(self, x: torch.Tensor, source: torch.Tensor, alpha, keep: Optional[torch.Tensor] = None, *,
                    noise: Optional[torch.Tensor] = None, noise_scale: float = 1.0, seed: int, clip_offset: int = 0,
                    index: int) -> torch.Tensor:
        if x.dim() < 2:
            raise ValueError("x must be [N, ..., T]")
        source, keep = check_keep_args(x, source, keep, 0, 1)
        _native.require_cuda(x, source, keep, noise)
        if noise is not None:
            if tuple(noise.shape) != tuple(x.shape):
                raise ValueError(f"noise of shape {tuple(noise.shape)} does not match the state's {tuple(x.shape)}")
            noise = noise.detach().to(torch.float32).contiguous()
        if not torch.is_tensor(alpha):
            alpha = torch.full((x.shape[0],), float(alpha), dtype=torch.float32)
        alpha = alpha.detach().to(device=x.device, dtype=torch.float32).reshape(-1).contiguous()
        if alpha.numel() == 1:
            alpha = alpha.expand(x.shape[0]).contiguous()
        if alpha.shape != (x.shape[0],):
            raise ValueError(f"alpha must hold one value or one per row ({x.shape[0]}), got {alpha.numel()}")
        out = x.detach().to(torch.float32).contiguous().clone()
        self._keep_(out, source, keep, alpha, noise=noise, noise_scale=noise_scale, seed=seed, clip_offset=clip_offset, index=index)
        return out.view_as(x)

    @staticmethod
    def _keep_(x, source, keep, alpha, *, noise=None, noise_scale=1.0, seed, clip_offset, index) -> None:
        B, T = x.shape[0], x[0].numel()
        with torch.cuda.device(x.device):
            _native.check(_native.lib().vqvs_keep_region(x.data_ptr(), source.data_ptr(), _native._ptr(keep), _native._ptr(noise),
                                                         alpha.data_ptr(), B, T, float(noise_scale), int(seed), int(clip_offset), int(index),
                                                         _native._stream_ptr()))

    def _keep_start(self, x_T, source, keep, alpha, *, start_step, seed, clip_offset) -> torch.Tensor:
        if start_step > 0:
            x, keep = torch.empty_like(source), None
        elif keep is None:
            return x_T
        else:
            x = x_T.detach().to(torch.float32).contiguous().clone()
        self._keep_(x, source, keep, alpha, seed=seed, clip_offset=clip_offset, index=start_step)
        return x.view_as(x_T)

    def _sample(self, what: str, layout, x_T: torch.Tensor, steps: int, *, schedule, noise: NoiseSource, seed, clip_offset, progress, source,
                keep, start_step) -> torch.Tensor:
        source, keep = check_keep_args(x_T, source, keep, start_step, steps)
        _native.require_cuda(x_T, source, keep)
        rows = layout.rows(x_T)
        if seed is None:
            seed = fresh_seed()
        key = dict(seed=seed, clip_offset=clip_offset)
        rule, predictor, cond_fn = layout.rule, layout.predictor, layout.cond_fn
        stack = few_guided_steps_promotion(what, steps, predictor, cond_fn, stacklevel=4)
        with stack if stack is not None else contextlib.nullcontext():
            if rule.name != "ddpm":
                warn_few_unguided_steps(what, steps, predictor, cond_fn, stacklevel=4)
            tables = self.step_tables(steps, rows, schedule, x_T.device)
            x_t = layout.start(x_T, source, keep, tables[1][start_step], start_step=start_step, **key)
            with torch.no_grad(), torch.cuda.device(x_T.device):
                for i in _progress(range(start_step, steps), progress):
                    last = i + 1 == steps
                    eps = layout.predict(x_t, tables, i)
                    nz = None
                    if not last and noise is not None and rule.draws_noise:
                        nz = noise(i) if callable(noise) else noise[i]
                    x_t = layout.step(x_t, eps, nz, tables, i, noise_scale=0.0 if last else 1.0, **key)
                    if keep is not None:
                        layout.keep(x_t, source, keep, tables[2][i], index=i + 1, **key)
            x_t = x_t.view_as(x_T)
            self.check_sample(predictor, x_t, what)
        return x_t

    def ddpm_sample_windows(self, x_T_long: torch.Tensor, predictor: Callable, steps: int, **kwargs) -> torch.Tensor:
        from .longform import ddpm_sample_windows

        return ddpm_sample_windows(self, x_T_long, predictor, steps, **kwargs)

    def ddpm_sample(
        self,
        x_T: torch.Tensor,
        predictor: Callable[[torch.Tensor, torch.Tensor], torch.Tensor],
        steps: int,
        progress: bool = False,
        sigma_large: bool = False,
        constrain: bool = False,
        cond_fn: Optional[Callable] = None,
        schedule: Optional[Callable] = None,
        *,
        noise: NoiseSource = None,
        seed: Optional[int] = None,
        clip_offset: int = 0,
        source: Optional[torch.Tensor] = None,
        keep: Optional[torch.Tensor] = None,
        start_step: int = 0,
    ) -> torch.Tensor:
        return self._sample("ddpm_sample", _Clips(self, _Ddpm(sigma_large, constrain), predictor, cond_fn), x_T, steps, schedule=schedule,
                            noise=noise, seed=seed, clip_offset=clip_offset, progress=progress, source=source, keep=keep,
                            start_step=start_step)

    def ddim_previous(
        self,
        x_t: torch.Tensor,
        ts: torch.Tensor,
        step,
        epsilon_prediction: torch.Tensor,
        noise: Optional[torch.Tensor] = None,
        eta: float = 0.0,
        constrain: bool = False,
        cond_fn: Optional[Callable] = None,
        *,
        seed: int = 0,
        clip_offset: int = 0,
        step_index: int = 0,
        noise_scale: float = 1.0,
    ) -> torch.Tensor:
        _native.require_cuda(x_t, epsilon_prediction, noise)
        ts = ts.detach().to(device=x_t.device, dtype=torch.float32)
        if not torch.is_tensor(step):
            step = torch.full_like(ts, float(step))
        step = step.to(ts)
        return self._ddim_step(x_t, epsilon_prediction, self.schedule(ts).contiguous(), self.schedule(ts - step).contiguous(), ts,
                               noise=noise, eta=eta, constrain=constrain, cond_fn=cond_fn, seed=seed, clip_offset=clip_offset,
                               step_index=step_index, noise_scale=noise_scale)

    def _ddim_step(self, x_t, epsilon_prediction, a_t, a_to, ts, *, noise=None, eta=0.0, constrain=False, cond_fn=None, invert=False,
                   seed=0, clip_offset=0, step_index=0, noise_scale=1.0) -> torch.Tensor:
        if x_t.dim() < 2:
            raise ValueError("x_t must be [N, ..., T]")
        B = x_t.shape[0]
        T = x_t[0].numel()
        x = x_t.detach().to(torch.float32).contiguous()
        eps = epsilon_prediction.detach().to(torch.float32).contiguous()
        flags = (_native.DDIM_CONSTRAIN if constrain else 0) | (_native.DDIM_INVERT if invert else 0)
        with torch.cuda.device(x.device):
            grad = None
            if cond_fn is not None:
                grad = cond_fn(x.view_as(x_t), ts).detach().to(torch.float32).contiguous()
                _native.require_cuda(grad)
                if grad.numel() != x.numel():
                    raise ValueError(f"cond_fn returned shape {tuple(grad.shape)} for a state of shape {tuple(x_t.shape)}")
            if noise is not None:
                noise = noise.detach().to(torch.float32).contiguous()
# ... 96 lines not shown
            _native.check(_native.lib().vqvs_dpmpp_step(x.data_ptr(), eps.data_ptr(), _native._ptr(grad), _native._ptr(x0_prev),
                                                        _native._ptr(a_from), a_t.data_ptr(), a_to.data_ptr(), out.data_ptr(), x0.data_ptr(),
                                                        B, T, _native.DDIM_CONSTRAIN if constrain else 0, _native._stream_ptr()))
        return out.view_as(x_t), x0.view_as(x_t)

    def dpmpp_sample(
        self,
        x_T: torch.Tensor,
        predictor: Callable[[torch.Tensor, torch.Tensor], torch.Tensor],
        steps: int,
        progress: bool = False,
        constrain: bool = False,
        cond_fn: Optional[Callable] = None,
        schedule: Optional[Callable] = None,
        *,
        noise: NoiseSource = None,
        seed: Optional[int] = None,
        clip_offset: int = 0,
        source: Optional[torch.Tensor] = None,
        keep: Optional[torch.Tensor] = None,
        start_step: int = 0,
    ) -> torch.Tensor:
        return self._sample("dpmpp_sample", _Clips(self, _Dpmpp(constrain), predictor, cond_fn), x_T, steps, schedule=schedule,
                            noise=noise, seed=seed, clip_offset=clip_offset, progress=progress, source=source, keep=keep,
                            start_step=start_step)

    def dpmpp_sample_windows(self, x_T_long: torch.Tensor, predictor: Callable, steps: int, **kwargs) -> torch.Tensor:
        from .longform import dpmpp_sample_windows

        return dpmpp_sample_windows(self, x_T_long, predictor, steps, **kwargs)


class _Ddpm:
    name, draws_noise = "ddpm", True

    def __init__(self, sigma_large: bool, constrain: bool):
        self.sigma_large, self.constrain = sigma_large, constrain
        self.flags = (_native.DDPM_SIGMA_LARGE if sigma_large else 0) | (_native.DDPM_CONSTRAIN if constrain else 0)

    def step(self, diffusion, x_t, eps, tables, i, **kw):
        _, a_t, a_prev, ts_prev = tables
        return diffusion._step(x_t, eps, a_t[i], a_prev[i], ts_prev[i], sigma_large=self.sigma_large, constrain=self.constrain, **kw)


class _Ddim:
    name = "ddim"

    def __init__(self, eta: float, constrain: bool):
        self.eta, self.constrain, self.draws_noise = eta, constrain, bool(eta)
        self.flags = _native.DDIM_CONSTRAIN if constrain else 0

    def step(self, diffusion, x_t, eps, tables, i, **kw):
        ts, a_t, a_to, _ = tables
        return diffusion._ddim_step(x_t, eps, a_t[i], a_to[i], ts[i], eta=self.eta, constrain=self.constrain, **kw)


class _Dpmpp:
    name, draws_noise = "dpmpp", False

    def __init__(self, constrain: bool):
        self.constrain = constrain
        self.flags = _native.DDIM_CONSTRAIN if constrain else 0
        self.x0_prev = self.a_from = None

    def step(self, diffusion, x_t, eps, tables, i, *, cond_fn=None, **noise_keys):
        ts, a_t, a_to, _ = tables
        x_to, self.x0_prev = diffusion._dpmpp_step(x_t, eps, self.a_from, a_t[i], a_to[i], ts[i], x0_prev=self.x0_prev,
                                                   constrain=self.constrain, cond_fn=cond_fn)
        self.a_from = a_t[i]
        return x_to


class _Clips:

    def __init__(self, diffusion: Diffusion, rule, predictor: Callable, cond_fn: Optional[Callable]):
        self.diffusion, self.rule, self.predictor, self.cond_fn = diffusion, rule, predictor, cond_fn

    def rows(self, x_T) -> int:
        return x_T.shape[0]

    def start(self, x_T, source, keep, alpha, **kw):
        return x_T if source is None else self.diffusion._keep_start(x_T, source, keep, alpha, **kw)

    def predict(self, x_t, tables, i):
        return self.predictor(x_t, tables[0][i])

    def step(self, x_t, eps, nz, tables, i, **kw):
        _native.require_cuda(eps, nz)
        return self.rule.step(self.diffusion, x_t, eps, tables, i, noise=nz, cond_fn=self.cond_fn, step_index=i, **kw)

    def keep(self, x_t, source, keep, alpha, **kw) -> None:
        self.diffusion._keep_(x_t, source, keep, alpha, **kw)


def randn_clips(n: int, T: int, device, seed: int, clip_offset: int = 0, stream_id: int = 1) -> torch.Tensor:
    out = torch.empty(n, 1, T, device=device, dtype=torch.float32)
    _native.require_cuda(out)
    with torch.cuda.device(out.device):
        _native.check(_native.lib().vqvs_randn(out.data_ptr(), n, T, int(seed), int(clip_offset), int(stream_id), _native._stream_ptr()))
    return out
```

vq_voice_swap_amd/longform.py:

```python

from __future__ import annotations

from typing import Callable, Optional, Tuple

import torch

from . import _native

MAX_WINDOWS = 65535


def plan_windows(num_samples: int, window: int, hop: int) -> Tuple[int, int]:
    num_samples, window, hop = int(num_samples), int(window), int(hop)
    if num_samples < 1:
        raise ValueError(f"num_samples={num_samples} must be at least 1")
    if window < 4 or hop < 4 or window % 4 or hop % 4:
        raise ValueError(f"window={window} and hop={hop} must be positive multiples of 4")
    overlap = window - hop
    if overlap < 0 or overlap > hop:
        raise ValueError(f"overlap {overlap} (window {window} - hop {hop}) must lie in 0..hop: at most two windows may cover a sample")
    n = 1 if num_samples <= window else -(-(num_samples - overlap) // hop)
    padded_len = (n - 1) * hop + window
    if n > MAX_WINDOWS or padded_len >= 2 ** 31:
        raise ValueError(f"{num_samples} samples need {n} windows spanning {padded_len} samples: more than {MAX_WINDOWS} windows or 2^31 samples")
# ... 28 lines not shown
    pad = (0, padded_len - num_samples)
    if source is not None:
        source = torch.nn.functional.pad(source, pad)
    if keep is not None:
        if keep.dtype not in (torch.bool, torch.uint8):
            raise ValueError(f"keep must be a bool or uint8 tensor, got {keep.dtype}")
        keep = torch.nn.functional.pad(keep.to(torch.uint8), pad)
    return source, keep


def _ddpm_fill(rule, xw, e, tables, i, b0, cond_fn, eps, grad, st) -> None:
    m, window = xw.shape[0], xw.shape[-1]
    e = e.detach().to(torch.float32).contiguous()
    if cond_fn is None:
        eps[b0:b0 + m].copy_(e)
        return
    L = _native.lib()
    a_t, a_prev = tables[1][i, :m], tables[2][i, :m]
    mean = torch.empty_like(xw)
    _native.check(L.vqvs_ddpm_mean(xw.data_ptr(), e.data_ptr(), a_t.data_ptr(), a_prev.data_ptr(), mean.data_ptr(), m, window, st))
    g = cond_fn(mean, tables[3][i, :m], first=b0).detach().to(torch.float32).contiguous()
    _native.check(L.vqvs_ddpm_guided_eps(xw.data_ptr(), mean.data_ptr(), g.data_ptr(), a_t.data_ptr(), a_prev.data_ptr(),
                                         eps[b0:b0 + m].data_ptr(), m, window, rule.flags, st))


def _ddim_fill(rule, xw, e, tables, i, b0, cond_fn, eps, grad, st) -> None:
    m = xw.shape[0]
    eps[b0:b0 + m].copy_(e.detach())
    if cond_fn is not None:
        g = cond_fn(xw, tables[0][i, :m], first=b0)
        _native.require_cuda(g)
        if tuple(g.shape) != tuple(xw.shape):
            raise ValueError(f"cond_fn returned shape {tuple(g.shape)} for windows of shape {tuple(xw.shape)}")
        grad[b0:b0 + m].copy_(g.detach())


def _ddpm_step_windows(rule, x, eps, grad, nz, a_t, a_to, x_to, next_windows, n, window, hop, noise_scale, seed, clip_offset, step_index, st) -> None:
    _native.check(_native.lib().vqvs_ddpm_step_windows(x.data_ptr(), eps.data_ptr(), _native._ptr(nz), a_t.data_ptr(), a_to.data_ptr(),
                                                       x_to.data_ptr(), next_windows.data_ptr(), n, window, hop, rule.flags, noise_scale,
                                                       int(seed), int(clip_offset), step_index, st))


def _ddim_step_windows(rule, x, eps, grad, nz, a_t, a_to, x_to, next_windows, n, window, hop, noise_scale, seed, clip_offset, step_index, st) -> None:
    _native.check(_native.lib().vqvs_ddim_step_windows(x.data_ptr(), eps.data_ptr(), _native._ptr(grad), _native._ptr(nz), a_t.data_ptr(),
                                                       a_to.data_ptr(), x_to.data_ptr(), next_windows.data_ptr(), n, window, hop,
                                                       rule.flags, float(rule.eta), noise_scale, int(seed), int(clip_offset), step_index, st))


def dpmpp_step_windows_(x, eps, grad, x0_prev, a_from, a_t, a_to, x_to, x0_out, next_windows, n, window, hop, flags, st) -> None:
    _native.check(_native.lib().vqvs_dpmpp_step_windows(x.data_ptr(), eps.data_ptr(), _native._ptr(grad), _native._ptr(x0_prev), _native._ptr(a_from),
                                                        a_t.data_ptr(), a_to.data_ptr(), x_to.data_ptr(), x0_out.data_ptr(),
                                                        next_windows.data_ptr(), n, window, hop, flags, st))


def _dpmpp_step_windows(rule, x, eps, grad, nz, a_t, a_to, x_to, next_windows, n, window, hop, noise_scale, seed, clip_offset, step_index, st) -> None:
    x0 = torch.empty_like(x)
    dpmpp_step_windows_(x, eps, grad, rule.x0_prev, rule.a_from, a_t, a_to, x_to, x0, next_windows, n, window, hop, rule.flags, st)
    rule.x0_prev, rule.a_from = x0, a_t


class _Windows:

    def __init__(self, rule, predictor: Callable, cond_fn: Optional[Callable], window: int, hop: int, window_batch: int, fill, step):
        self.rule, self.predictor, self.cond_fn, self.fill, self.step_windows = rule, predictor, cond_fn, fill, step
        self.window, self.hop, self.window_batch = window, hop, window_batch

    def rows(self, x_T_long) -> int:
        if x_T_long.dim() != 3 or x_T_long.shape[0] != 1 or x_T_long.shape[1] != 1:
            raise ValueError(f"x_T_long must be [1, 1, Np], got {tuple(x_T_long.shape)}")
        self.Np = x_T_long.shape[2]
        self.n, padded = plan_windows(self.Np, self.window, self.hop)
        if padded != self.Np:
            raise ValueError(f"x_T_long has {self.Np} samples: {self.n} windows of {self.window} every {self.hop} span {padded} (see plan_windows)")
        if self.window_batch < 1:
            raise ValueError(f"window_batch={self.window_batch} must be at least 1")
        self.mb = min(self.n, int(self.window_batch))
        return self.mb

    def start(self, x_T_long, source, keep, alpha, **kw):
        x, self.windows = start_windows(x_T_long, source, keep, alpha, n=self.n, window=self.window, hop=self.hop, **kw)
        self.eps = torch.empty_like(self.windows)
        self.grad = torch.empty_like(self.windows) if self.cond_fn is not None and self.rule.name != "ddpm" else None
        return x

    def predict(self, x, tables, i) -> None:
        self.st = _native._stream_ptr()
        for b0 in range(0, self.n, self.mb):
            m = min(self.mb, self.n - b0)
            xw = self.windows[b0:b0 + m]
            e = self.predictor(xw, tables[0][i, :m], first=b0)
            _native.require_cuda(e)
            if tuple(e.shape) != tuple(xw.shape):
                raise ValueError(f"the predictor returned shape {tuple(e.shape)} for windows of shape {tuple(xw.shape)}")
            self.fill(self.rule, xw, e, tables, i, b0, self.cond_fn, self.eps, self.grad, self.st)

    def step(self, x, _, nz, tables, i, *, noise_scale, seed, clip_offset):
        if nz is not None:
            _native.require_cuda(nz)
            nz = nz.detach().to(torch.float32).contiguous()
            if nz.numel() != self.Np:
                raise ValueError(f"noise of step {i} has {nz.numel()} values: expected [1, 1, {self.Np}]")
        x_to, next_windows = torch.empty_like(x), torch.empty_like(self.windows)
        self.step_windows(self.rule, x, self.eps, self.grad, nz, tables[1][i], tables[2][i], x_to, next_windows, self.n, self.window, self.hop,
                          noise_scale, seed, clip_offset, i, self.st)
        self.windows = next_windows
        return x_to

    def keep(self, x, source, keep, alpha, **kw) -> None:
        keep_windows_(x, self.windows, source, keep, alpha, n=self.n, window=self.window, hop=self.hop, **kw)


def ddpm_sample_windows(diffusion, x_T_long: torch.Tensor, predictor: Callable, steps: int, *, window: int, hop: int,
                        window_batch: int = 64, constrain: bool = False, sigma_large: bool = False, cond_fn: Optional[Callable] = None,
                        schedule: Optional[Callable] = None, noise=None, seed: Optional[int] = None, clip_offset: int = 0,
                        progress: bool = False, source: Optional[torch.Tensor] = None, keep: Optional[torch.Tensor] = None,
                        start_step: int = 0) -> torch.Tensor:
    from .diffusion import _Ddpm

    layout = _Windows(_Ddpm(sigma_large, constrain), predictor, cond_fn, window, hop, window_batch, _ddpm_fill, _ddpm_step_windows)
    return diffusion._sample("ddpm_sample_windows", layout, x_T_long, steps, schedule=schedule, noise=noise, seed=seed, clip_offset=clip_offset,
                             progress=progress, source=source, keep=keep, start_step=start_step)


def ddim_sample_windows(diffusion, x_T_long: torch.Tensor, predictor: Callable, steps: int, *, window: int, hop: int,
                        window_batch: int = 64, eta: float = 0.0, constrain: bool = False, cond_fn: Optional[Callable] = None,
                        schedule: Optional[Callable] = None, noise=None, seed: Optional[int] = None, clip_offset: int = 0,
                        progress: bool = False, source: Optional[torch.Tensor] = None, keep: Optional[torch.Tensor] = None,
                        start_step: int = 0) -> torch.Tensor:
    from .diffusion import _Ddim

    layout = _Windows(_Ddim(eta, constrain), predictor, cond_fn, window, hop, window_batch, _ddim_fill, _ddim_step_windows)
    return diffusion._sample("ddim_sample_windows", layout, x_T_long, steps, schedule=schedule, noise=noise, seed=seed, clip_offset=clip_offset,
                             progress=progress, source=source, keep=keep, start_step=start_step)


def dpmpp_sample_windows(diffusion, x_T_long: torch.Tensor, predictor: Callable, steps: int, *, window: int, hop: int,
                         window_batch: int = 64, constrain: bool = False, cond_fn: Optional[Callable] = None,
                         schedule: Optional[Callable] = None, noise=None, seed: Optional[int] = None, clip_offset: int = 0,
                         progress: bool = False, source: Optional[torch.Tensor] = None, keep: Optional[torch.Tensor] = None,
                         start_step: int = 0) -> torch.Tensor:
    from .diffusion import _Dpmpp

    layout = _Windows(_Dpmpp(constrain), predictor, cond_fn, window, hop, window_batch, _ddim_fill, _dpmpp_step_windows)
    return diffusion._sample("dpmpp_sample_windows", layout, x_T_long, steps, schedule=schedule, noise=noise, seed=seed, clip_offset=clip_offset,
                             progress=progress, source=source, keep=keep, start_step=start_step)


def encode_long(model, wave: torch.Tensor, window: int, hop: int, window_batch: int = 64) -> torch.Tensor:
    if wave.dim() != 3 or wave.shape[0] != 1 or wave.shape[1] != 1:
        raise ValueError(f"wave must be [1, 1, N], got {tuple(wave.shape)}")
    check_rate(model, window, hop)
    n, padded = plan_windows(wave.shape[2], window, hop)
    windows = gather_windows(torch.nn.functional.pad(wave, (0, padded - wave.shape[2])), window, hop)
    mb = 1 if getattr(model.encoder, "version", 1) == 2 else max(1, int(window_batch))
    return torch.cat([model.encode(windows[b0:b0 + mb]) for b0 in range(0, n, mb)])


def check_rate(model, window: int, hop: int) -> None:
    rate = model.downsample_rate
    if window % rate or hop % rate:
        raise ValueError(f"window={window} and hop={hop} must be multiples of the model's downsample rate {rate}")


def decode_long(model, codes: torch.Tensor, labels: Optional[torch.Tensor] = None, *, num_samples: int, window: int, hop: int,
                steps: int = 100, progress: bool = False, constrain: bool = False, enc_pred=None, enc_pred_scale: float = 1.0,
                seed: Optional[int] = None, clip_offset: int = 0, window_batch: int = 64, sampler: str = "ddpm", eta: float = 0.0,
# ... 44 lines not shown
```

vq_voice_swap_amd/unet.py:

```python

from __future__ import annotations

import contextlib
import functools
import os
import warnings
from typing import Callable, List, Optional, Tuple

import torch
import torch.nn as nn

from . import _native

CHANNEL_MULT = (1, 1, 2, 2, 2, 4, 4, 8, 8)
MIDDLE_DILATIONS = (4, 8, 16, 32)


SUPPORTED_BASE_CHANNELS = (32, 64, 128)


def pad_blocks(base_channels: int) -> Tuple[int, int]:
    k = 0
    while (base_channels >> k) & 1 == 0 and k < 5:
        k += 1
# ... 46 lines not shown

def check_topology(base_channels: int, channel_mult, depth_mult: int, dilations) -> None:
    if not 1 <= len(channel_mult) <= 12:
        raise ValueError(f"channel_mult must have 1..12 entries (got {len(channel_mult)})")
    for m in channel_mult:
        if int(m) != m or m < 1 or (m * base_channels) % 32 or m * base_channels > 1024:
            raise ValueError(f"channel_mult entry {m}: widths must be multiples of 32 in base_channels..1024")
    if int(depth_mult) != depth_mult or not 1 <= depth_mult <= 8:
        raise ValueError(f"depth_mult must be an integer in 1..8 (got {depth_mult})")
    if len(dilations) > 12 or any(int(d) != d or not 1 <= d <= 32 for d in dilations):
        raise ValueError(f"dilations must be at most 12 integers in 1..32 (got {tuple(dilations)})")


def default_precision() -> str:
    return os.environ.get("VQVS_PRECISION", "fp32")


def _groups(ch: int) -> int:
    g = 32
    while ch % g:
        g //= 2
    return g


def _scaled(mod: nn.Module, s: float) -> nn.Module:
    with torch.no_grad():
        for p in mod.parameters():
            p.mul_(s)
    return mod


class _Slot(nn.Module):

    def forward(self, x):
        return x


def _seq(*mods: Optional[nn.Module]) -> nn.Sequential:
    return nn.Sequential(*[m if m is not None else _Slot() for m in mods])


class ResBlock(nn.Module):

    def __init__(self, channels: int, emb_channels: Optional[int] = None, out_channels: Optional[int] = None,
                 scale_factor: float = 1.0, dilation: int = 2, dropout: float = 0.0):
        super().__init__()
        self.channels = channels
        self.emb_channels = emb_channels
        self.out_channels = out_channels or channels
        self.scale_factor = scale_factor
        self.dilation = dilation
        self.dropout = dropout
        co = self.out_channels
        self.skip = _seq(None, nn.Conv1d(channels, co, 1) if channels != co else None)
        if emb_channels:
            self.cond_layers = _seq(None, _scaled(nn.Linear(emb_channels, 2 * co), 0.1))
        self.pre_cond = _seq(_seq(nn.GroupNorm(_groups(channels), channels), None), None,
                             nn.Conv1d(channels, co, 3, padding=1), nn.GroupNorm(_groups(co), co))
        conv2 = _scaled(nn.Conv1d(co, co, 3, padding=dilation, dilation=dilation), 0.0)
        self.post_cond = _seq(None, None, conv2) if dropout else _seq(None, conv2)


class _NativeModule(nn.Module):

    def __init__(self):
        super().__init__()
        self._handle = None
        self._handle_key = None
        self.precision = default_precision()
        self.debug_taps = False

    def set_precision(self, precision: str):
        if precision not in _native.PRECISIONS:
            raise ValueError(f"unknown precision {precision!r}; use 'fp32', 'fp16' or 'bf16'")
        self.precision = precision
        self.invalidate()
        return self

    def invalidate(self):
        if self._handle is not None:
            self._handle.close()
        self._handle = None
        self._handle_key = None
        for h, _ in self.__dict__.pop("_alt_handles", {}).values():
            if h is not None:
                h.close()
        for h in self.__dict__.pop("_cond_handles", {}).values():
            h.close()

    COND_HANDLES_KEPT = 3

    ALT_HANDLE_KEEP_BYTES = int(float(os.environ.get("VQVS_ALT_HANDLE_KEEP_GB", "2")) * 2 ** 30)

    @contextlib.contextmanager
    def precision_override(self, precision: str):
        if precision not in _native.PRECISIONS:
            raise ValueError(f"unknown precision {precision!r}; use 'fp32', 'fp16' or 'bf16'")
        if precision == self.precision:
            yield self
            return
        own = (self.precision, self._handle, self._handle_key)
        alt = self.__dict__.setdefault("_alt_handles", {})
        h, k = alt.pop(precision, (None, None))
        self.precision, self._handle, self._handle_key = precision, h, k
        try:
            yield self
        finally:
            alt = self.__dict__.setdefault("_alt_handles", {})
            stale = alt.pop(precision, (None, None))[0]
            if stale is not None and stale is not self._handle:
                stale.close()
            if self._handle is not None and self._handle.device_bytes() > self.ALT_HANDLE_KEEP_BYTES:
                self._handle.close()
            elif self._handle is not None:
                alt[precision] = (self._handle, self._handle_key)
            self.precision, self._handle, self._handle_key = own

    def release_alt_handles(self):
        for h, _ in self.__dict__.pop("_alt_handles", {}).values():
            if h is not None:
                h.close()

    def _apply(self, fn, *a, **k):
        self.invalidate()
        return super()._apply(fn, *a, **k)

    def load_state_dict(self, *a, **k):
        self.invalidate()
        return super().load_state_dict(*a, **k)

    def _load_from_state_dict(self, *a, **k):
        self.invalidate()
        return super()._load_from_state_dict(*a, **k)

    def _cfg(self) -> _native.Cfg:
        raise NotImplementedError

    def _weights_token(self):
        tok = 0
        for t in list(self.parameters()) + list(self.buffers()):
            tok = (tok * 1000003 + t._version * 8191 + t.data_ptr() + id(t)) & 0xFFFFFFFFFFFF
        return tok

    def check_status(self) -> None:
        handles = [h for h in (self._handle, self.__dict__.get("_alt_handles", {}).get("grad", (None, None))[0]) if h is not None]
        if not handles:
            return
        w = 0
        for h in handles:
            w |= h.status()
        if w & 1:
            raise _native.NativeError("range guard: non-finite GroupNorm statistics (an activation overflowed the storage type, or the "
                                      "input held NaN/inf); run this model with set_precision('fp32')")
        if w & 2:
            msg = ("range guard: a tile's sum of squares reached 9e8 in the fp16 mode (an activation may be near fp16's limit of 65504); "
                   "consider set_precision('fp32')")
            if os.environ.get("VQVS_STRICT_RANGE", "0") == "1":
                raise _native.NativeError(msg)
            warnings.warn(msg, RuntimeWarning, stacklevel=2)

    def handle(self, device: torch.device, B: int, T: int) -> _native.Handle:
        idx = device.index if device.index is not None else torch.cuda.current_device()
        key = (idx, self.precision, bool(self.debug_taps), self._weights_token(), getattr(self, "_cond_code", 0))
        h = self._handle
        if h is not None and self._handle_key == key and h.cfg.max_batch >= B and h.cfg.max_T >= T:
            return h
        if h is not None and self._handle_key[:4] == key[:4] and self._handle_key != key:
            kept = self.__dict__.setdefault("_cond_handles", {})
            if h.device_bytes() <= self.ALT_HANDLE_KEEP_BYTES:
                kept[self._handle_key] = h
                while len(kept) > self.COND_HANDLES_KEPT:
                    kept.pop(next(iter(kept))).close()
            else:
                h.close()
            self._handle, self._handle_key = None, None
            back = kept.pop(key, None)
            if back is not None and back.cfg.max_batch >= B and back.cfg.max_T >= T:
                self._handle, self._handle_key = back, key
                return back
            if back is not None:
                B, T = max(B, back.cfg.max_batch), max(T, back.cfg.max_T)
                back.close()
            h = None
        if h is not None:
            same_shape_class = self._handle_key[:3] == key[:3]
            B = max(B, h.cfg.max_batch) if same_shape_class else B
            T = max(T, h.cfg.max_T) if same_shape_class else T
            self.invalidate()
        cfg = self._cfg()
        cfg.precision = _native.PRECISIONS[self.precision]
        cfg.max_batch = B
        cfg.max_T = T
        cfg.debug_taps = 1 if self.debug_taps else 0
        torch.cuda.synchronize(idx)
        state = self.state_dict()
        q, qp = pad_blocks(getattr(self, "base_channels", 32)) if cfg.reserved[4] else (1, 1)
        if q != qp:
            state = pad_state(state, _native.param_table(cfg), q, qp)
        self._handle = _native.Handle(cfg, state, "", idx)
        self._handle_key = key
        return self._handle

    def __getstate__(self):
        d = self.__dict__.copy()
        d["_handle"] = None
        d["_handle_key"] = None
        d.pop("_token_tensors", None)
        d.pop("_alt_handles", None)
        d.pop("_cond_handles", None)
        return d

    def __deepcopy__(self, memo):
        import copy

        cls = self.__class__
        new = cls.__new__(cls)
        memo[id(self)] = new
        for k, v in self.__dict__.items():
            if k in ("_token_tensors", "_alt_handles", "_cond_handles"):
                continue
            new.__dict__[k] = None if k in ("_handle", "_handle_key") else copy.deepcopy(v, memo)
        return new

    def _check_inference_only(self, *tensors):
        if torch.is_grad_enabled() and any(t is not None and t.requires_grad for t in tensors):
            import warnings

            warnings.warn("the gfx950 UNet path is inference-only: inputs are detached, no gradient flows through forward()",
                          RuntimeWarning, stacklevel=3)
        if self.training and getattr(self, "dropout", 0.0):
            raise RuntimeError("the gfx950 UNet path does not implement dropout: call .eval() before sampling "
                               "(the reference applies dropout only in training, unet.py:295-300)")


class UNetPredictor(_NativeModule):
    def __init__(self, base_channels: int, channel_mult: Tuple[int, ...] = CHANNEL_MULT,
                 middle_dilations: Tuple[int, ...] = MIDDLE_DILATIONS, depth_mult: int = 2,
                 cond_channels: Optional[int] = None, num_labels: Optional[int] = None,
                 in_channels: int = 1, out_channels: int = 1, dropout: float = 0.0):
        super().__init__()
        check_base_channels(base_channels, pad_ok=True)
        check_topology(physical_base(base_channels), tuple(channel_mult), depth_mult, tuple(middle_dilations))
        if channel_mult[0] != 1:
            raise ValueError("channel_mult[0] must be 1: the output head (GroupNorm + conv) is built for base_channels")
        self.base_channels = base_channels
        self.channel_mult = tuple(channel_mult)
        self.middle_dilations = tuple(middle_dilations)
        self.depth_mult = depth_mult
        self.cond_channels = cond_channels
        self.num_labels = num_labels
        self.in_channels = in_channels
        self.out_channels = out_channels
        self.dropout = dropout
        self._cond_code = 0

        C = base_channels
        E = 4 * C
        self.time_embed = nn.Module()
        self.time_embed.proj = nn.Linear(E, E)
        self.time_embed.channels = E
        self.time_embed_extra = _seq(None, nn.Linear(E, E))
        if num_labels is not None:
            self.class_embed = nn.Embedding(num_labels, E)
        if cond_channels is not None:
            self.cond_proj = nn.Conv1d(cond_channels, C, 3, padding=1)
        self.in_conv = nn.Conv1d(in_channels, C, 3, padding=1)

        down, stack, cur = [], [C], C
        last = len(channel_mult) - 1
        for depth, mult in enumerate(channel_mult):
            for _ in range(depth_mult):
                down.append(ResBlock(cur, E, mult * C, dropout=dropout))
                cur = mult * C
                stack.append(cur)
            if depth != last:
                down.append(ResBlock(cur, E, scale_factor=0.5, dropout=dropout))
                stack.append(cur)
        self.down_blocks = nn.ModuleList(down)
        self.middle_blocks = nn.ModuleList([ResBlock(cur, E, dilation=d, dropout=dropout) for d in middle_dilations])
        up = []
        for depth in range(last, -1, -1):
            mult = channel_mult[depth]
            for _ in range(depth_mult + 1):
                up.append(ResBlock(cur + stack.pop(), E, mult * C, dropout=dropout))
                cur = mult * C
            if depth:
                up.append(ResBlock(cur, E, scale_factor=2.0, dropout=dropout))
        self.up_blocks = nn.ModuleList(up)
        self.out = _seq(_seq(nn.GroupNorm(_groups(C), C), None), nn.Conv1d(C, out_channels, 3, padding=1))

    def _cfg(self) -> _native.Cfg:
        cfg = _native.Cfg()
        cfg.kind = _native.KIND_PREDICTOR
        cfg.base_channels = physical_base(self.base_channels)
        cfg.reserved[4] = self.base_channels if cfg.base_channels != self.base_channels else 0
        cfg.in_channels = self.in_channels
        cfg.out_channels = self.out_channels
        cfg.cond_channels = self.cond_channels or 0
        cfg.num_labels = self.num_labels or 0
        cfg.reserved[0] = 1 if self.dropout else 0
        cfg.reserved[3] = self._cond_code
        if (self.channel_mult, self.middle_dilations, self.depth_mult) != (CHANNEL_MULT, MIDDLE_DILATIONS, 2):
            cfg.set_topology(self.channel_mult, self.depth_mult, self.middle_dilations)
        return cfg

    def forward(self, x: torch.Tensor, ts: torch.Tensor, cond: Optional[torch.Tensor] = None,
                labels: Optional[torch.Tensor] = None, use_checkpoint: bool = False) -> torch.Tensor:
        assert (labels is None) == (self.num_labels is None), "must provide labels if and only if model is class conditional"
        assert (cond is None) == (self.cond_channels is None), "must provide cond sequence if and only if model is conditional"
        _native.require_cuda(x, ts, cond, labels)
        self._check_inference_only(x, cond)
        if x.dim() != 3 or x.shape[1] != self.in_channels:
            raise ValueError(f"expected x of shape [N, {self.in_channels}, T], got {tuple(x.shape)}")
        B, _, T = x.shape
        if T % self.downsample_rate:
            raise ValueError(f"T={T} is not a multiple of the UNet downsample rate {self.downsample_rate}")
        x = x.detach().to(torch.float32).contiguous()
        ts = ts.detach().to(device=x.device, dtype=torch.float32).contiguous()
        if ts.shape != (B,):
            raise ValueError(f"expected ts of shape [{B}], got {tuple(ts.shape)}")
        if cond is not None:
            cond = cond.detach().to(torch.float32).contiguous()
            if tuple(cond.shape[:2]) != (B, self.cond_channels) or cond.shape[2] < 1:
                raise ValueError(f"expected cond of shape {(B, self.cond_channels)} x L, got {tuple(cond.shape)}")
            lens = {(T // 160 + 1 - 2) // 2 + 1: 1, T // 256: 0}
            code = lens.get(cond.shape[2], 1000 + cond.shape[2])
            self._cond_code = code
        if labels is not None:
            labels = labels.detach().to(device=x.device, dtype=torch.int64).contiguous()
            if labels.shape != (B,):
                raise ValueError(f"expected labels of shape [{B}], got {tuple(labels.shape)}")
            _native.check_index_range(labels, self.num_labels, "class labels")
        h = self.handle(x.device, B, T)
        out = torch.empty(B, self.out_channels, T, device=x.device, dtype=torch.float32)
        with torch.cuda.device(x.device):
            _native.check(_native.lib().vqvs_unet_forward(
                h.ptr, x.data_ptr(), ts.data_ptr(), _native._ptr(cond), _native._ptr(labels), out.data_ptr(), B, T,
                _native._stream_ptr()))
        return out

    def condition(self, **kwargs) -> Callable:
        return functools.partial(self, **kwargs)

    def add_labels(self, n: int, end: bool = True):
        assert self.num_labels is not None
        old = self.class_embed.weight.detach()
        count = self.num_labels
        self.num_labels += n
        self.class_embed = nn.Embedding(self.num_labels, old.shape[-1]).to(old.device)
        with torch.no_grad():
            if end:
                self.class_embed.weight[:count].copy_(old)
            else:
                self.class_embed.weight[n:].copy_(old)
        self.invalidate()

    def label_parameters(self) -> List[nn.Parameter]:
        assert self.num_labels is not None
        return list(self.class_embed.parameters())

    def _grad_handle(self, device: torch.device, B: int, T: int) -> _native.Handle:
        if self.out_channels != 1:
            raise ValueError(f"embedding_grad: out_channels={self.out_channels}: the loss is the MSE of a one-channel noise prediction")
        if physical_base(self.base_channels) != self.base_channels:
            raise ValueError(f"embedding_grad: base_channels={self.base_channels} is a padded width; the gradient schedule is built for multiples of 32")
        idx = device.index if device.index is not None else torch.cuda.current_device()
        key = (idx, self._weights_token(), self._cond_code)
        alt = self.__dict__.setdefault("_alt_handles", {})
        h, k = alt.get("grad", (None, None))
        if h is not None and k == key and h.cfg.max_batch >= B and h.cfg.max_T >= T:
            return h
        if h is not None:
            if k == key:
                B, T = max(B, h.cfg.max_batch), max(T, h.cfg.max_T)
            h.close()
            del alt["grad"]
        cfg = self._cfg()
        cfg.kind = _native.KIND_PREDICTOR_GRAD
        cfg.precision = _native.PREC_F32
        cfg.max_batch = B
        cfg.max_T = T
        torch.cuda.synchronize(idx)
        h = _native.Handle(cfg, self.state_dict(), "", idx)
        alt["grad"] = (h, key)
        return h

    def embedding_grad(self, x_t: torch.Tensor, ts: torch.Tensor, eps: torch.Tensor, vectors: torch.Tensor, *,
                       cond: Optional[torch.Tensor] = None, return_pred: bool = False):
        assert self.num_labels is not None, "embedding_grad needs a class-conditional model"
        assert (cond is None) == (self.cond_channels is None), "must provide cond sequence if and only if model is conditional"
        _native.require_cuda(x_t, ts, eps, vectors, cond)
        if x_t.dim() != 3 or x_t.shape[1] != self.in_channels:
            raise ValueError(f"expected x_t of shape [N, {self.in_channels}, T], got {tuple(x_t.shape)}")
        B, _, T = x_t.shape
        if T % self.downsample_rate:
            raise ValueError(f"T={T} is not a multiple of the UNet downsample rate {self.downsample_rate}")
        E = 4 * self.base_channels
        x_t = x_t.detach().to(torch.float32).contiguous()
        ts = ts.detach().to(device=x_t.device, dtype=torch.float32).contiguous()
        eps = eps.detach().to(torch.float32).contiguous()
        vectors = vectors.detach().to(device=x_t.device, dtype=torch.float32).contiguous()
        if ts.shape != (B,) or tuple(eps.shape) != (B, 1, T) or tuple(vectors.shape) != (B, E):
            raise ValueError(f"expected ts [{B}], eps [{B}, 1, {T}] and vectors [{B}, {E}], got {tuple(ts.shape)}, {tuple(eps.shape)}, {tuple(vectors.shape)}")
        if cond is not None:
            cond = cond.detach().to(torch.float32).contiguous()
            if tuple(cond.shape[:2]) != (B, self.cond_channels) or cond.shape[2] < 1:
                raise ValueError(f"expected cond of shape {(B, self.cond_channels)} x L, got {tuple(cond.shape)}")
            lens = {(T // 160 + 1 - 2) // 2 + 1: 1, T // 256: 0}
            self._cond_code = lens.get(cond.shape[2], 1000 + cond.shape[2])
        h = self._grad_handle(x_t.device, B, T)
        mses = torch.empty(B, device=x_t.device, dtype=torch.float32)
        grads = torch.empty(B, E, device=x_t.device, dtype=torch.float32)
        pred = torch.empty(B, 1, T, device=x_t.device, dtype=torch.float32) if return_pred else None
        with torch.cuda.device(x_t.device):
            _native.check(_native.lib().vqvs_unet_embed_grad(
                h.ptr, x_t.data_ptr(), ts.data_ptr(), _native._ptr(cond), vectors.data_ptr(), eps.data_ptr(), mses.data_ptr(),
                grads.data_ptr(), _native._ptr(pred), B, T, _native._stream_ptr()))
        return (mses, grads, pred) if return_pred else (mses, grads)

    @property
    def downsample_rate(self) -> int:
# ... 96 lines not shown
```

Measured before the change: 68.91 clips/s.

## Precompute per-step time embedding and FiLM tables before the sampling loop

```diff
diff --git a/include/vqvs.h b/include/vqvs.h
--- a/include/vqvs.h
+++ b/include/vqvs.h
@@ -59,6 +59,11 @@
 
 int vqvs_unet_forward(vqvs_model* m, const float* d_x, const float* d_ts, const float* d_cond,
                       const int64_t* d_labels, float* d_out, int B, int T, void* stream);
+
+#define VQVS_PREPARED_STEPS_MAX_BYTES (64 << 20)
+int vqvs_unet_prepare_steps(vqvs_model* m, const float* d_ts, int nsteps, int clip_stride, const int64_t* d_labels, int B, int T,
+                            int64_t max_bytes, void* stream);
+int vqvs_unet_forward_step(vqvs_model* m, const float* d_x, int step, const float* d_cond, float* d_out, int B, int T, void* stream);
 
 int vqvs_encoder_forward(vqvs_model* m, const float* d_x, float* d_z, int B, int T, void* stream);
 
diff --git a/vq_voice_swap_amd/_native.py b/vq_voice_swap_amd/_native.py
--- a/vq_voice_swap_amd/_native.py
+++ b/vq_voice_swap_amd/_native.py
@@ -66,6 +66,7 @@
     "vqvs_debug_tap_info", "vqvs_debug_tap_rows", "vqvs_debug_read_tap", "vqvs_debug_read_embedding", "vqvs_forward_kernel_count", "vqvs_forward_model_bytes",
     "vqvs_forward_flops", "vqvs_set_profiling", "vqvs_op_info", "vqvs_op_desc", "vqvs_profile_read", "vqvs_last_error", "vqvs_version",
     "vqvs_unet_embed_grad", "vqvs_embed_adamw", "vqvs_debug_read_dfilm", "vqvs_head_xent_grad", "vqvs_head_adamw",
+    "vqvs_unet_prepare_steps", "vqvs_unet_forward_step",
 ]
 
 _lib = None
@@ -119,6 +120,8 @@
     L.vqvs_model_device_bytes.argtypes = [vp]
     L.vqvs_model_device_bytes.restype = i64
     L.vqvs_unet_forward.argtypes = [vp, vp, vp, vp, vp, vp, i32, i32, vp]
+    L.vqvs_unet_prepare_steps.argtypes = [vp, vp, i32, i32, vp, i32, i32, i64, vp]
+    L.vqvs_unet_forward_step.argtypes = [vp, vp, i32, vp, vp, i32, i32, vp]
     L.vqvs_unet_embed_grad.argtypes = [vp, vp, vp, vp, vp, vp, vp, vp, vp, i32, i32, vp]
     L.vqvs_embed_adamw.argtypes = [vp, vp, vp, vp, vp, i32, i32, i32, i32, f32, f32, f32, f32, f32, vp]
     L.vqvs_debug_read_dfilm.argtypes = [vp, i32, vp]
diff --git a/vq_voice_swap_amd/csrc/api.cpp b/vq_voice_swap_amd/csrc/api.cpp
--- a/vq_voice_swap_amd/csrc/api.cpp
+++ b/vq_voice_swap_amd/csrc/api.cpp
@@ -147,6 +147,7 @@
   for (auto e : m->events) (void)hipEventDestroy(e);
   if (m->d_weights) (void)hipFree(m->d_weights);
   if (m->d_arena) (void)hipFree(m->d_arena);
+  if (m->prep.d) (void)hipFree(m->prep.d);
   delete m;
 }
 
@@ -180,6 +181,65 @@
   c.labels = d_labels;
   c.out = d_out;
   c.st = reinterpret_cast<hipStream_t>(stream);
+  m->emb_src = nullptr;
+  return run_model(m, c);
+}
+
+int vqvs_unet_prepare_steps(vqvs_model* m, const float* d_ts, int nsteps, int clip_stride, const int64_t* d_labels, int B, int T,
+                            int64_t max_bytes, void* stream) {
+  if (int e = check_run(m, VQVS_KIND_PREDICTOR, B, T)) return e;
+  m->prep.nsteps = 0;
+  m->emb_src = nullptr;
+  if (!d_ts) VQVS_FAIL(VQVS_ERR_ARG, "ts must be non-NULL");
+  if (nsteps < 1 || nsteps > 65535) VQVS_FAIL(VQVS_ERR_ARG, "nsteps %d outside 1..65535", nsteps);
+  if (clip_stride != 0 && clip_stride != 1) VQVS_FAIL(VQVS_ERR_ARG, "clip_stride %d: 0 (one t per step) or 1 (ts is [nsteps][B])", clip_stride);
+  if ((d_labels == nullptr) != (m->cfg.num_labels == 0)) VQVS_FAIL(VQVS_ERR_ARG, "must provide labels if and only if model is class conditional");
+  if (!m->prepare_rows) VQVS_FAIL(VQVS_ERR_STATE, "this handle has no prepared-steps form");
+  const int Bc = clip_stride == 0 && !d_labels ? 1 : B;
+  const int64_t rows = (int64_t)nsteps * Bc;
+  const int64_t floats = rows * (m->film_R + 2 * m->emb_E);
+  const int64_t cap = max_bytes > 0 ? max_bytes : (int64_t)VQVS_PREPARED_STEPS_MAX_BYTES;
+  if (floats * 4 > cap || rows > 65535 * 32) return 0;
+  if ((size_t)floats > m->prep.cap_floats) {
+    if (m->prep.d) VQVS_HIP(hipFree(m->prep.d));
+    m->prep.d = nullptr;
+    m->prep.cap_floats = 0;
+    VQVS_HIP(hipMalloc(&m->prep.d, (size_t)floats * 4));
+    m->prep.cap_floats = (size_t)floats;
+  }
+  float* film = m->prep.d;
+  float* emb = film + rows * m->film_R;
+  float* gemb = emb + rows * m->emb_E;
+  if (int e = m->prepare_rows(d_ts, clip_stride ? B : 1, clip_stride, d_labels, (int)rows, Bc, film, emb, gemb,
+                              reinterpret_cast<hipStream_t>(stream)))
+    return e;
+  m->prep.nsteps = nsteps;
+  m->prep.Bc = Bc;
+  m->prep.B = B;
+  m->prep.T = T;
+  return 1;
+}
+
+int vqvs_unet_forward_step(vqvs_model* m, const float* d_x, int step, const float* d_cond, float* d_out, int B, int T, void* stream) {
+  if (int e = check_run(m, VQVS_KIND_PREDICTOR, B, T)) return e;
+  if (!d_x || !d_out) VQVS_FAIL(VQVS_ERR_ARG, "x and out must be non-NULL");
+  if ((d_cond == nullptr) != (m->cfg.cond_channels == 0)) VQVS_FAIL(VQVS_ERR_ARG, "must provide cond sequence if and only if model is conditional");
+  const auto& p = m->prep;
+  if (!p.nsteps) VQVS_FAIL(VQVS_ERR_STATE, "no steps are prepared (vqvs_unet_prepare_steps)");
+  if (B != p.B || T != p.T) VQVS_FAIL(VQVS_ERR_STATE, "steps were prepared for %d clips of %d samples, not %d of %d", p.B, p.T, B, T);
+  if (step < 0 || step >= p.nsteps) VQVS_FAIL(VQVS_ERR_ARG, "step %d outside the %d prepared", step, p.nsteps);
+  const size_t rows = (size_t)p.nsteps * p.Bc;
+  RunCtx c;
+  c.B = B;
+  c.Lbase = T;
+  c.x = d_x;
+  c.cond = d_cond;
+  c.out = d_out;
+  c.film_tab = p.d + (size_t)step * p.Bc * m->film_R;
+  c.film_tab_stride = p.Bc == 1 ? 0 : m->film_R;
+  c.st = reinterpret_cast<hipStream_t>(stream);
+  m->emb_src = p.d + rows * m->film_R + (size_t)step * p.Bc * m->emb_E;
+  m->emb_src_stride = p.Bc == 1 ? 0 : m->emb_E;
   return run_model(m, c);
 }
 
@@ -761,6 +821,11 @@
   if (!m->emb_E) VQVS_FAIL(VQVS_ERR_STATE, "this model kind has no timestep embedding");
   VQVS_HIP(hipSetDevice(m->device));
   VQVS_HIP(hipDeviceSynchronize());
+  if (m->emb_src) {
+    for (int b = 0; b < B; ++b)
+      VQVS_HIP(hipMemcpy(h_out + (size_t)b * m->emb_E, m->emb_src + (size_t)b * m->emb_src_stride, m->emb_E * sizeof(float), hipMemcpyDeviceToHost));
+    return m->emb_E;
+  }
   const float* src = reinterpret_cast<const float*>(m->d_arena + m->misc_off) + m->emb_misc_off;
   VQVS_HIP(hipMemcpy(h_out, src, (size_t)B * m->emb_E * sizeof(float), hipMemcpyDeviceToHost));
   return m->emb_E;
diff --git a/vq_voice_swap_amd/csrc/kernels.hpp b/vq_voice_swap_amd/csrc/kernels.hpp
--- a/vq_voice_swap_amd/csrc/kernels.hpp
+++ b/vq_voice_swap_amd/csrc/kernels.hpp
@@ -115,6 +115,7 @@
   float* emb;
   float* gemb;
   int E;
+  int rows_per_step, ts_step_stride, ts_clip_stride;
 };
 int launch_time_embed(const TimeEmbedArgs& a, int B, hipStream_t st);
 int launch_gelu_rows(const float* in, float* out, int n, hipStream_t st);
diff --git a/vq_voice_swap_amd/csrc/misc_kernels.hip b/vq_voice_swap_amd/csrc/misc_kernels.hip
--- a/vq_voice_swap_amd/csrc/misc_kernels.hip
+++ b/vq_voice_swap_amd/csrc/misc_kernels.hip
@@ -77,6 +77,74 @@
     float* o = a.stats + (((size_t)b * a.ntiles + blockIdx.x) * a.C + tid) * 2;
     o[0] = t1;
     o[1] = t2;
+  }
+}
+
+template <typename T>
+__global__ __launch_bounds__(256) void in_conv_stream_kernel(const InConvArgs a, int tiles_total, int per) {
+  __shared__ float red[256 * 8 * 2];
+  __shared__ float xs[STAT_TILE + 2];
+  const int tid = threadIdx.x;
+  const int opr = a.C >> 3;
+  const int rpp = 256 / opr;
+  const int oct = tid % opr;
+  const int r0 = tid / opr;
+  const int c = oct * 8;
+  float w0[8], w1[8], w2[8], bs[8];
+#pragma unroll
+  for (int j = 0; j < 8; ++j) {
+    w0[j] = a.w[(c + j) * 3 + 0];
+    w1[j] = a.w[(c + j) * 3 + 1];
+    w2[j] = a.w[(c + j) * 3 + 2];
+    bs[j] = a.bias[c + j];
+  }
+  const bool active = r0 < rpp;
+  const float cond_scale = a.condp ? (float)a.cond_len / (float)a.T : 0.f;
+  const int tile_end = min(tiles_total, ((int)blockIdx.x + 1) * per);
+  for (int tile = blockIdx.x * per; tile < tile_end; ++tile) {
+    const int b = tile / a.ntiles, tx = tile - b * a.ntiles;
+    const int t0 = tx * STAT_TILE;
+    const float* xb = a.x + (size_t)b * a.T;
+    for (int i = tid; i < STAT_TILE + 2; i += 256) {
+      const int t = t0 - 1 + i;
+      xs[i] = t >= 0 && t < a.T ? xb[t] : 0.f;
+    }
+    __syncthreads();
+    f32x8 s1 = f32x8_zero(), s2 = f32x8_zero();
+    if (active) {
+      const int nr = min(STAT_TILE, a.T - t0);
+      for (int r = r0; r < nr; r += rpp) {
+        const int t = t0 + r;
+        const float xm = xs[r], x0 = xs[r + 1], xp = xs[r + 2];
+        f32x8 v;
+#pragma unroll
+        for (int j = 0; j < 8; ++j) v[j] = fmaf(w2[j], xp, fmaf(w1[j], x0, fmaf(w0[j], xm, bs[j])));
+        if (a.condp) {
+          const int cr = min((int)floorf((float)t * cond_scale), a.cond_len - 1);
+          const T* cp = reinterpret_cast<const T*>(a.condp) + ((size_t)b * a.cond_len + cr) * a.C + c;
+          v += Elem<T>::load8(cp);
+        }
+        s1 += v;
+        s2 += v * v;
+        Elem<T>::store8(reinterpret_cast<T*>(a.out) + ((size_t)b * a.T + t) * a.C + c, v);
+      }
+#pragma unroll
+      for (int j = 0; j < 8; ++j) {
+        red[(r0 * a.C + c + j) * 2 + 0] = s1[j];
+        red[(r0 * a.C + c + j) * 2 + 1] = s2[j];
+      }
+    }
+    __syncthreads();
+    if (tid < a.C) {
+      float t1 = 0.f, t2 = 0.f;
+      for (int g = 0; g < rpp; ++g) {
+        t1 += red[(g * a.C + tid) * 2 + 0];
+        t2 += red[(g * a.C + tid) * 2 + 1];
+      }
+      float* o = a.stats + (((size_t)b * a.ntiles + tx) * a.C + tid) * 2;
+      o[0] = t1;
+      o[1] = t2;
+    }
   }
 }
 
@@ -280,7 +348,13 @@
   const int tid = threadIdx.x;
   const int b = blockIdx.x;
   const int E = a.E, half = E >> 1;
-  const float t = a.ts[b];
+  int clip = b, tb = b;
+  if (a.rows_per_step > 0) {
+    const int step = b / a.rows_per_step;
+    clip = b - step * a.rows_per_step;
+    tb = step * a.ts_step_stride + clip * a.ts_clip_stride;
+  }
+  const float t = a.ts[tb];
   for (int j = tid; j < half; j += 256) {
     const float arg = t * a.freqs[j];
     e0[j] = cosf(arg);
@@ -300,7 +374,7 @@
   __syncthreads();
   const float* ce = nullptr;
   if (a.class_embed) {
-    long long lab = a.labels[b];
+    long long lab = a.labels[clip];
     if (lab < 0) lab = 0;
     if (lab >= a.num_labels) lab = a.num_labels - 1;
     ce = a.class_embed + (size_t)lab * E;
@@ -315,7 +389,7 @@
     }
     float v = (acc0 + acc1) + (acc2 + acc3) + a.b2[r];
     if (ce) v += ce[r];
-    if (a.class_vec) v += a.class_vec[(size_t)b * E + r];
+    if (a.class_vec) v += a.class_vec[(size_t)clip * E + r];
     a.emb[(size_t)b * E + r] = v;
     a.gemb[(size_t)b * E + r] = gelu_f(v);
   }
@@ -466,6 +540,14 @@
   }
 }
 
+struct StreamGrid {
+  int blocks, tiles, per;
+};
+StreamGrid stream_grid(long long tiles) {
+  const int per = (int)((tiles + 2047) / 2048);
+  return StreamGrid{(int)((tiles + per - 1) / per), (int)tiles, per};
+}
+
 }
 
 int launch_in_conv(const InConvArgs& a, int B, int precision, hipStream_t st) {
@@ -474,7 +556,9 @@
   if (a.Cin > 1) {
     VQVS_BY_PRECISION(precision, hipLaunchKernelGGL((in_conv_kernel<T, true>), grid, dim3(256), 0, st, a));
   } else {
-    VQVS_BY_PRECISION(precision, hipLaunchKernelGGL((in_conv_kernel<T, false>), grid, dim3(256), 0, st, a));
+    if ((long long)grid.x * B >= (1ll << 31)) VQVS_FAIL(-1, "in_conv: %lld tiles", (long long)grid.x * B);
+    const StreamGrid g = stream_grid((long long)grid.x * B);
+    VQVS_BY_PRECISION(precision, hipLaunchKernelGGL(in_conv_stream_kernel<T>, dim3(g.blocks), dim3(256), 0, st, a, g.tiles, g.per));
   }
   VQVS_HIP(hipGetLastError());
   return 0;
@@ -518,6 +602,7 @@
 
 int launch_film(const FilmArgs& a, int B, hipStream_t st) {
   if (a.E > 1024 || a.E < 32 || a.E % 32) VQVS_FAIL(-1, "film: unsupported E=%d", a.E);
+  if (B < 1 || (B + FILM_NB - 1) / FILM_NB > 65535) VQVS_FAIL(-1, "film: %d rows outside 1..%d", B, 65535 * FILM_NB);
   const int lds = (a.E * FILM_NB + 3 * 64 * (FILM_NB + 1)) * 4;
   static std::atomic<bool> attr_done[64];
   int dev = 0;
diff --git a/vq_voice_swap_amd/csrc/net.cpp b/vq_voice_swap_amd/csrc/net.cpp
--- a/vq_voice_swap_amd/csrc/net.cpp
+++ b/vq_voice_swap_amd/csrc/net.cpp
@@ -335,8 +335,8 @@
       a.inv_count = 1.0 / ((double)(Creal / groups) * (double)L);
       a.gamma = reinterpret_cast<const float*>(self->wp(g_off));
       a.beta = reinterpret_cast<const float*>(self->wp(b_off));
-      a.film = film ? self->miscp(film_misc_off) : nullptr;
-      a.film_stride = film_stride;
+      a.film = !film ? nullptr : c.film_tab ? c.film_tab : self->miscp(film_misc_off);
+      a.film_stride = film && c.film_tab ? c.film_tab_stride : film_stride;
       a.film_off = film_off;
       a.ss = reinterpret_cast<float2*>(self->ssp(ss_off));
       a.mr = want_mr ? reinterpret_cast<float2*>(self->ssp(mr_off)) : nullptr;
@@ -1155,21 +1155,26 @@
     m->emb_E = E;
     const int NL = c.num_labels;
     m->meta.push_back({"time_embed", "", 0, 0, 0});
-    m->add_op([=](const RunCtx& r) -> int {
+    auto time_embed_args = [=]() {
       TimeEmbedArgs a{};
-      a.ts = r.ts;
       a.freqs = reinterpret_cast<const float*>(bp->wp(freq_off));
       a.w1 = reinterpret_cast<const float*>(bp->wp(w1));
       a.b1 = reinterpret_cast<const float*>(bp->wp(b1));
       a.w2 = reinterpret_cast<const float*>(bp->wp(w2));
       a.b2 = reinterpret_cast<const float*>(bp->wp(b2));
       a.class_embed = NL > 0 && !gradk ? reinterpret_cast<const float*>(bp->wp(ce)) : nullptr;
+      a.num_labels = NL;
+      a.E = E;
+      return a;
+    };
+    m->add_op([=](const RunCtx& r) -> int {
+      if (r.film_tab) return 0;
+      TimeEmbedArgs a = time_embed_args();
+      a.ts = r.ts;
       a.labels = r.labels;
       a.class_vec = gradk ? r.class_vec : nullptr;
-      a.num_labels = NL;
       a.emb = bp->miscp(emb_off);
       a.gemb = bp->miscp(gemb_off);
-      a.E = E;
       return launch_time_embed(a, r.B, r.st);
     });
     std::vector<const BlockSpec*> all;
@@ -1193,10 +1198,28 @@
     const size_t film_off = b.alloc_misc((size_t)c.max_batch * R);
     m->meta.push_back({"film", "", 0, 0, 0});
     m->add_op([=](const RunCtx& r) -> int {
+      if (r.film_tab) return 0;
       FilmArgs f{bp->miscp(gemb_off), reinterpret_cast<const float*>(bp->wp(wall_off)), reinterpret_cast<const float*>(bp->wp(ball_off)),
                  bp->miscp(film_off), E, R};
       return launch_film(f, r.B, r.st);
     });
+    if (c.kind == VQVS_KIND_PREDICTOR) {
+      m->film_R = R;
+      m->prepare_rows = [=](const float* ts, int ts_step_stride, int ts_clip_stride, const int64_t* labels, int rows, int Bc, float* film,
+                            float* emb, float* gemb, hipStream_t st) -> int {
+        TimeEmbedArgs a = time_embed_args();
+        a.ts = ts;
+        a.labels = labels;
+        a.emb = emb;
+        a.gemb = gemb;
+        a.rows_per_step = Bc;
+        a.ts_step_stride = ts_step_stride;
+        a.ts_clip_stride = ts_clip_stride;
+        if (int e = launch_time_embed(a, rows, st)) return e;
+        FilmArgs f{gemb, reinterpret_cast<const float*>(bp->wp(wall_off)), reinterpret_cast<const float*>(bp->wp(ball_off)), film, E, R};
+        return launch_film(f, rows, st);
+      };
+    }
     TensorH condp{};
     const bool has_cond = c.cond_channels > 0;
     if (has_cond) {
diff --git a/vq_voice_swap_amd/csrc/net.hpp b/vq_voice_swap_amd/csrc/net.hpp
--- a/vq_voice_swap_amd/csrc/net.hpp
+++ b/vq_voice_swap_amd/csrc/net.hpp
@@ -47,6 +47,8 @@
   float* feat = nullptr;
   float* probs = nullptr;
   const float* class_vec = nullptr;
+  const float* film_tab = nullptr;
+  int film_tab_stride = 0;
   const float* eps = nullptr;
   float* mse = nullptr;
   float* egrad = nullptr;
@@ -96,6 +98,16 @@
   size_t status_misc_off = (size_t)-1;
   size_t emb_misc_off = 0;
   int emb_E = 0;
+  struct PreparedSteps {
+    float* d = nullptr;
+    size_t cap_floats = 0;
+    int nsteps = 0, Bc = 0, B = 0, T = 0;
+  } prep;
+  int film_R = 0;
+  std::function<int(const float* ts, int ts_step_stride, int ts_clip_stride, const int64_t* labels, int rows, int Bc, float* film,
+                    float* emb, float* gemb, hipStream_t st)> prepare_rows;
+  const float* emb_src = nullptr;
+  int emb_src_stride = 0;
   size_t dfilm_misc_off = 0;
   int dfilm_R = 0;
   std::shared_ptr<void> keepalive;
diff --git a/vq_voice_swap_amd/diffusion.py b/vq_voice_swap_amd/diffusion.py
--- a/vq_voice_swap_amd/diffusion.py
+++ b/vq_voice_swap_amd/diffusion.py
@@ -2,8 +2,10 @@
 from __future__ import annotations
 
 import contextlib
+import functools
 import math
 import operator
+import os
 from typing import Callable, List, Optional, Sequence, Union
 
 import torch
@@ -64,6 +66,18 @@
     for m in getattr(fn, "native_modules", ()) or ():
         add(m)
     return out
+
+
+PREPARE_STEPS = os.environ.get("VQVS_PREPARED_STEPS", "1") != "0"
+
+
+def prepare_predictor_steps(predictor, ts: torch.Tensor, x: torch.Tensor) -> bool:
+    mod, kw = predictor, {}
+    if isinstance(predictor, functools.partial) and not predictor.args:
+        mod, kw = predictor.func, predictor.keywords
+    if not PREPARE_STEPS or not hasattr(mod, "prepare_steps") or set(kw) - {"cond", "labels"}:
+        return False
+    return bool(mod.prepare_steps(ts, x, **kw))
 
 
 def predictor_check_status(predictor):
@@ -412,6 +426,7 @@
             tables = self.step_tables(steps, rows, schedule, x_T.device)
             x_t = layout.start(x_T, source, keep, tables[1][start_step], start_step=start_step, **key)
             with torch.no_grad(), torch.cuda.device(x_T.device):
+                layout.prepare(x_t, tables)
                 for i in _progress(range(start_step, steps), progress):
                     last = i + 1 == steps
                     eps = layout.predict(x_t, tables, i)
@@ -674,7 +689,12 @@
     def start(self, x_T, source, keep, alpha, **kw):
         return x_T if source is None else self.diffusion._keep_start(x_T, source, keep, alpha, **kw)
 
+    def prepare(self, x_t, tables) -> None:
+        self.prepared = prepare_predictor_steps(self.predictor, tables[0][:, 0], x_t)
+
     def predict(self, x_t, tables, i):
+        if self.prepared:
+            return self.predictor(x_t, tables[0][i], step=i)
         return self.predictor(x_t, tables[0][i])
 
     def step(self, x_t, eps, nz, tables, i, **kw):
diff --git a/vq_voice_swap_amd/longform.py b/vq_voice_swap_amd/longform.py
--- a/vq_voice_swap_amd/longform.py
+++ b/vq_voice_swap_amd/longform.py
@@ -134,6 +134,10 @@
         self.eps = torch.empty_like(self.windows)
         self.grad = torch.empty_like(self.windows) if self.cond_fn is not None and self.rule.name != "ddpm" else None
         return x
+
+    def prepare(self, x, tables) -> None:
+        """Nothing: the predictor of a window loop is a callable over slices (`first=`), each with its own rows of the conditioning;
+        every slice computes its embedding and FiLM rows per step, as before."""
 
     def predict(self, x, tables, i) -> None:
         self.st = _native._stream_ptr()
diff --git a/vq_voice_swap_amd/unet.py b/vq_voice_swap_amd/unet.py
--- a/vq_voice_swap_amd/unet.py
+++ b/vq_voice_swap_amd/unet.py
@@ -152,6 +152,7 @@
             self._handle.close()
         self._handle = None
         self._handle_key = None
+        self.__dict__.pop("_prepared", None)
         for h, _ in self.__dict__.pop("_alt_handles", {}).values():
             if h is not None:
                 h.close()
@@ -278,6 +279,7 @@
         d.pop("_token_tensors", None)
         d.pop("_alt_handles", None)
         d.pop("_cond_handles", None)
+        d.pop("_prepared", None)
         return d
 
     def __deepcopy__(self, memo):
@@ -287,7 +289,7 @@
         new = cls.__new__(cls)
         memo[id(self)] = new
         for k, v in self.__dict__.items():
-            if k in ("_token_tensors", "_alt_handles", "_cond_handles"):
+            if k in ("_token_tensors", "_alt_handles", "_cond_handles", "_prepared"):
                 continue
             new.__dict__[k] = None if k in ("_handle", "_handle_key") else copy.deepcopy(v, memo)
         return new
@@ -374,8 +376,7 @@
             cfg.set_topology(self.channel_mult, self.depth_mult, self.middle_dilations)
         return cfg
 
-    def forward(self, x: torch.Tensor, ts: torch.Tensor, cond: Optional[torch.Tensor] = None,
-                labels: Optional[torch.Tensor] = None, use_checkpoint: bool = False) -> torch.Tensor:
+    def _conditioning(self, x: torch.Tensor, ts: torch.Tensor, cond: Optional[torch.Tensor], labels: Optional[torch.Tensor]):
         assert (labels is None) == (self.num_labels is None), "must provide labels if and only if model is class conditional"
         assert (cond is None) == (self.cond_channels is None), "must provide cond sequence if and only if model is conditional"
         _native.require_cuda(x, ts, cond, labels)
@@ -385,10 +386,6 @@
         B, _, T = x.shape
         if T % self.downsample_rate:
             raise ValueError(f"T={T} is not a multiple of the UNet downsample rate {self.downsample_rate}")
-        x = x.detach().to(torch.float32).contiguous()
-        ts = ts.detach().to(device=x.device, dtype=torch.float32).contiguous()
-        if ts.shape != (B,):
-            raise ValueError(f"expected ts of shape [{B}], got {tuple(ts.shape)}")
         if cond is not None:
             cond = cond.detach().to(torch.float32).contiguous()
             if tuple(cond.shape[:2]) != (B, self.cond_channels) or cond.shape[2] < 1:
@@ -401,12 +398,53 @@
             if labels.shape != (B,):
                 raise ValueError(f"expected labels of shape [{B}], got {tuple(labels.shape)}")
             _native.check_index_range(labels, self.num_labels, "class labels")
+        return B, T, cond, labels
+
+    PREPARED_STEPS_MAX_BYTES = 0
+
+    def prepare_steps(self, ts: torch.Tensor, x: torch.Tensor, cond: Optional[torch.Tensor] = None,
+                      labels: Optional[torch.Tensor] = None) -> bool:
+        labels_in = labels
+        B, T, cond, labels = self._conditioning(x, ts, cond, labels)
+        ts = ts.detach().to(device=x.device, dtype=torch.float32).contiguous()
+        if ts.dim() not in (1, 2) or (ts.dim() == 2 and ts.shape[1] != B) or ts.shape[0] < 1:
+            raise ValueError(f"expected ts of shape [steps] or [steps, {B}], got {tuple(ts.shape)}")
+        self._prepared = None
+        h = self.handle(x.device, B, T)
+        with torch.cuda.device(x.device):
+            rc = _native.lib().vqvs_unet_prepare_steps(h.ptr, ts.data_ptr(), ts.shape[0], ts.dim() - 1, _native._ptr(labels), B, T,
+                                                       int(self.PREPARED_STEPS_MAX_BYTES), _native._stream_ptr())
+        if rc < 0:
+            _native.check(rc)
+        if rc == 1:
+            self._prepared = (h, B, T, ts.shape[0], labels_in, None if labels_in is None else labels_in._version)
+        return rc == 1
+
+    def _prepared_step(self, h: _native.Handle, B: int, T: int, step: Optional[int], labels: Optional[torch.Tensor]) -> bool:
+        p = self.__dict__.get("_prepared")
+        if step is None or p is None:
+            return False
+        return (p[0] is h and p[0].ptr and (p[1], p[2]) == (B, T) and 0 <= step < p[3] and p[4] is labels
+                and (labels is None or labels._version == p[5]))
+
+    def forward(self, x: torch.Tensor, ts: torch.Tensor, cond: Optional[torch.Tensor] = None,
+                labels: Optional[torch.Tensor] = None, use_checkpoint: bool = False, step: Optional[int] = None) -> torch.Tensor:
+        labels_in = labels
+        B, T, cond, labels = self._conditioning(x, ts, cond, labels)
+        x = x.detach().to(torch.float32).contiguous()
+        ts = ts.detach().to(device=x.device, dtype=torch.float32).contiguous()
+        if ts.shape != (B,):
+            raise ValueError(f"expected ts of shape [{B}], got {tuple(ts.shape)}")
         h = self.handle(x.device, B, T)
         out = torch.empty(B, self.out_channels, T, device=x.device, dtype=torch.float32)
         with torch.cuda.device(x.device):
-            _native.check(_native.lib().vqvs_unet_forward(
-                h.ptr, x.data_ptr(), ts.data_ptr(), _native._ptr(cond), _native._ptr(labels), out.data_ptr(), B, T,
-                _native._stream_ptr()))
+            if self._prepared_step(h, B, T, step, labels_in):
+                _native.check(_native.lib().vqvs_unet_forward_step(h.ptr, x.data_ptr(), int(step), _native._ptr(cond), out.data_ptr(), B, T,
+                                                                   _native._stream_ptr()))
+            else:
+                _native.check(_native.lib().vqvs_unet_forward(
+                    h.ptr, x.data_ptr(), ts.data_ptr(), _native._ptr(cond), _native._ptr(labels), out.data_ptr(), B, T,
+                    _native._stream_ptr()))
         return out
 
     def condition(self, **kwargs) -> Callable:
```

Result: no change. 68.96 clips/s, median of 2 (+0.1%).
